# xguo7/SND-VAE

Measured on AMD Instinct MI355X. Metric: training graphs/sec + ELBO-step ms, N=4096 d=64, at 1/2/4/8 MI355X, higher is better.
Workload: dtype bf16; 1 GPU; C2: node-latent SND-VAE train step, N=4096, d=64, 8 graphs/GPU, HIP-graph replay; n_nodes=4096, latent=64, graphs_per_gpu=8, global_batch=8, parallelism=dp1, hip_graph=True

## Files before the change

snd_vae_amd/csrc/snd_common.hpp:

```cpp
#pragma once
#include <hip/hip_runtime.h>
#include <cstdint>
#include <cstdio>
#include <string>

#include "../../include/snd_vae.h"

namespace snd {

void set_error(const char* fmt, ...);

#define SND_CHECK_ARG(cond, ...)                                   \
  do {                                                             \
    if (!(cond)) {                                                 \
      ::snd::set_error(__VA_ARGS__);                               \
      return SND_ERR_ARG;                                          \
    }                                                              \
  } while (0)

#define SND_LAUNCH_CHECK(what)                                     \
  do {                                                             \
    hipError_t e_ = hipGetLastError();                             \
    if (e_ != hipSuccess) {                                        \
      ::snd::set_error("%s: %s", what, hipGetErrorString(e_));     \
// ... 25 lines not shown
inline int device_cu_count() {
  static const int n = [] {
    int d = 0, v = 0;
    if (hipGetDevice(&d) != hipSuccess ||
        hipDeviceGetAttribute(&v, hipDeviceAttributeMultiprocessorCount, d) != hipSuccess || v <= 0) {
      (void)hipGetLastError();
      return 256;
    }
    return v;
  }();
  return n;
}

__device__ __forceinline__ void edge_ce_terms(float x, float pw, float& coef, float& loss) {
  coef = -pw;
  if (pw != 1.f) {
    const float e = __expf(-fabsf(x));
    const float q = 1.f + e;
    const float r = __builtin_amdgcn_rcpf(q);
    const float sg = x >= 0.f ? r : e * r;
    coef += (pw - 1.f) * sg;
    loss += (pw - 1.f) * (fmaxf(x, 0.f) + __logf(q));
  }
}

__device__ __forceinline__ float kl_elem(float s, float mu) {
  const float x = 2.f * s;
  float r;
  if (fabsf(x) < 0.5f) {
    float t = 1.f / 3628800.f;
    t = __fmaf_rn(t, x, 1.f / 362880.f);
    t = __fmaf_rn(t, x, 1.f / 40320.f);
    t = __fmaf_rn(t, x, 1.f / 5040.f);
    t = __fmaf_rn(t, x, 1.f / 720.f);
    t = __fmaf_rn(t, x, 1.f / 120.f);
    t = __fmaf_rn(t, x, 1.f / 24.f);
    t = __fmaf_rn(t, x, 1.f / 6.f);
    t = __fmaf_rn(t, x, 0.5f);
    r = __fmul_rn(__fmul_rn(x, x), t);
  } else {
    r = __fsub_rn(__fsub_rn(__expf(x), 1.f), x);
  }
  return __fsub_rn(-r, __fmul_rn(mu, mu));
}

typedef __bf16 bf16x8 __attribute__((ext_vector_type(8)));
typedef __bf16 bf16x4 __attribute__((ext_vector_type(4)));
typedef float f32x4 __attribute__((ext_vector_type(4)));
typedef float f32x16 __attribute__((ext_vector_type(16)));
typedef unsigned u32x4 __attribute__((ext_vector_type(4)));

__device__ __forceinline__ float wave_sum(float v) {
#pragma unroll
  for (int o = 32; o > 0; o >>= 1) v += __shfl_xor(v, o, 64);
  return v;
}
__device__ __forceinline__ double wave_sum_d(double v) {
#pragma unroll
  for (int o = 32; o > 0; o >>= 1) v += __shfl_xor(v, o, 64);
  return v;
}
__device__ __forceinline__ unsigned wave_sum_u(unsigned v) {
#pragma unroll
  for (int o = 32; o > 0; o >>= 1) v += __shfl_xor(v, o, 64);
  return v;
}

template <int CTRL>
__device__ __forceinline__ float dpp_f(float v) {
  return __int_as_float(__builtin_amdgcn_update_dpp(0, __float_as_int(v), CTRL, 0xF, 0xF, true));
}
__device__ __forceinline__ float row8_sum(float v) {
  v += dpp_f<0xB1>(v);
  v += dpp_f<0x4E>(v);
  v += dpp_f<0x141>(v);
  return v;
}
__device__ __forceinline__ float row16_sum(float v) {
  v = row8_sum(v);
  v += dpp_f<0x140>(v);
  return v;
}

__device__ __forceinline__ uint4 philox4x32_10(uint4 c, uint2 k) {
  const unsigned M0 = 0xD2511F53u, M1 = 0xCD9E8D57u, W0 = 0x9E3779B9u, W1 = 0xBB67AE85u;
#pragma unroll
  for (int i = 0; i < 10; ++i) {
    const unsigned hi0 = __umulhi(M0, c.x), lo0 = M0 * c.x;
    const unsigned hi1 = __umulhi(M1, c.z), lo1 = M1 * c.z;
    c = make_uint4(hi1 ^ c.y ^ k.x, lo1, hi0 ^ c.w ^ k.y, lo0);
    k.x += W0;
    k.y += W1;
  }
  return c;
}

__device__ __forceinline__ float4 philox_normal4(unsigned long long seed, unsigned offset,
                                                unsigned long long q) {
  const uint4 r = philox4x32_10(make_uint4((unsigned)q, (unsigned)(q >> 32), offset, 0u),
                                make_uint2((unsigned)seed, (unsigned)(seed >> 32)));
  const float k = 2.3283064365386963e-10f;
  const float m1 = __builtin_amdgcn_sqrtf(-2.0f * __logf(((float)r.x + 1.0f) * k));
  const float m2 = __builtin_amdgcn_sqrtf(-2.0f * __logf(((float)r.z + 1.0f) * k));
  float s1, c1, s2, c2;
  __sincosf(6.283185307179586f * ((float)r.y * k), &s1, &c1);
  __sincosf(6.283185307179586f * ((float)r.w * k), &s2, &c2);
  return make_float4(m1 * c1, m1 * s1, m2 * c2, m2 * s2);
}

__device__ __forceinline__ float philox_normal(unsigned long long seed, unsigned offset,
                                               unsigned long long idx) {
  const float4 v = philox_normal4(seed, offset, idx >> 2);
  switch (idx & 3) {
    case 0: return v.x;
    case 1: return v.y;
    case 2: return v.z;
    default: return v.w;
  }
}

__device__ __forceinline__ void reparam_bwd_elem(float mu, float ls, float eps, float djd, float ej, float dzd,
                                                 float adj, float kl, float& dm, float& dl) {
  const float es = __expf(ls);
  const float dz = __fmaf_rn(adj, __fadd_rn(djd, ej), dzd);
  dm = __fmaf_rn(kl, mu, dz);
  dl = __fmaf_rn(__fmul_rn(dz, eps), es, __fmul_rn(kl, __fmaf_rn(es, es, -1.f)));
}

inline int cdiv(long long a, long long b) { return (int)((a + b - 1) / b); }
inline long long round_up(long long a, long long b) { return (a + b - 1) / b * b; }

__device__ __forceinline__ void adam_elem(float& p, float& m, float& v, float g, float b1, float b2,
                                          float eps, float lrt) {
  m = __fmaf_rn(b1, m, __fmul_rn(1.f - b1, g));
  v = __fmaf_rn(b2, v, __fmul_rn(__fmul_rn(1.f - b2, g), g));
  p = __fsub_rn(p, __fmul_rn(__fmul_rn(lrt, m),
                             __builtin_amdgcn_rcpf(__fadd_rn(__builtin_amdgcn_sqrtf(v), eps))));
}

}
```

snd_vae_amd/csrc/snd_elem.hip:

```cpp
#include "snd_elem.hpp"

#include <algorithm>
#include "snd_gemm.hpp"
#include "snd_tref.hpp"

namespace snd {
namespace {

template <typename T>
__device__ __forceinline__ T block_sum(T v) {
  __shared__ T sh[16];
  v = (sizeof(T) == 8) ? (T)wave_sum_d((double)v) : (T)wave_sum((float)v);
  const int w = threadIdx.x >> 6, nw = blockDim.x >> 6;
  if ((threadIdx.x & 63) == 0) sh[w] = v;
  __syncthreads();
  T t = 0;
  if (threadIdx.x == 0)
    for (int k = 0; k < nw; ++k) t += sh[k];
  return t;
}

constexpr int kReparamGrid = 2048;

__global__ void __launch_bounds__(256) reparam_fwd_kernel(ReparamFwdArgs a) {
// ... 261 lines not shown
#pragma unroll
      for (int k = 0; k < RG; ++k) {
        const int r = rb + k * RP;
        const bool rv = r < r1;
        dv[k] = rv ? a.dg[(long long)r * a.lddg + c] : 0.f;
        hv[k] = (rv && he) ? a.h2[(long long)r * a.ldh2 + c] : 0.f;
        pv[k] = (rv && hc) ? a.p[(long long)r * a.ldp + c] : 0.f;
      }
#pragma unroll
      for (int k = 0; k < RG; ++k) {
        const int r = rb + k * RP;
        if (r >= r1) break;
        float d = dv[k];
        if (he) {
          sge += d * hv[k];
          sbe += d;
          d *= gec;
        }
        if (hc) {
          sg += d * lrelu(pv[k]);
          sb += d;
          a.dp[(long long)r * a.lddp + c] = d * gc * lrelu_grad(pv[k]);
        }
      }
    }
  }
  if (a.has_enc) {
    sge = lane_rows_sum<CP>(sge, red);
    sbe = lane_rows_sum<CP>(sbe, red);
  }
  sg = lane_rows_sum<CP>(sg, red);
  sb = lane_rows_sum<CP>(sb, red);
  if (threadIdx.x < width) {
    const int stride = (a.has_enc ? 2 * a.wenc : 0) + 2 * a.h;
    float* pp = a.part + (long long)blockIdx.x * stride;
    int o = 0;
    if (a.has_enc) {
      pp[c] = sge * kBnC;
      pp[a.wenc + c] = sbe;
      o = 2 * a.wenc;
    }
    if (c < a.h) {
      pp[o + c] = sg * kBnC;
      pp[o + a.h + c] = sb;
    }
  }
}

#ifndef SND_RED_PL
#define SND_RED_PL 2
#endif
#ifndef SND_RED_PLS
#define SND_RED_PLS 4
#endif
#ifndef SND_RED_PLW
#define SND_RED_PLW 2
#endif
constexpr long long kRedWide = 2048;
__host__ __device__ __forceinline__ int red_pl(int nparts, long long items) {
  return nparts >= 1024 ? 64
                        : (nparts >= 256 ? 32 : (nparts >= 64 ? (items >= kRedWide ? SND_RED_PL : 8) : (items >= kRedWide ? SND_RED_PLW : SND_RED_PLS)));
}
struct ReducePack {
  ReduceDesc d[kMaxReduce];
  int bstart[kMaxReduce + 1];
};

template <int NTF> __device__ void finalize_block(const FinalizeArgs& a);

template <bool FIN, bool ADAM>
__global__ void __launch_bounds__(256) reduce_kernel(ReducePack pk, FinalizeArgs fin, ReduceAdam ra) {
  if constexpr (FIN) {
    if (blockIdx.x == 0) { finalize_block<256>(fin); return; }
  }
  const int bid = (int)blockIdx.x - (FIN ? 1 : 0);
  int di = 0;
#pragma unroll
  for (int i = 1; i < kMaxReduce; ++i) di += bid >= pk.bstart[i] ? 1 : 0;
  di = __builtin_amdgcn_readfirstlane(di);
  const ReduceDesc& d = pk.d[di];
  const int bx = bid - pk.bstart[di];
  const bool dad = ADAM && ((ra.mask >> di) & 1ull);
  float lrt = 0.f;
  if (dad) {
    const int st = *ra.stepn;
    lrt = (float)((double)ra.lr * sqrt(1.0 - pow((double)ra.b2, st)) / (1.0 - pow((double)ra.b1, st)));
  }
  __shared__ double red[256];
  const int rows = d.rows > 0 ? d.rows : 1;
  const long long items = (long long)rows * d.len;
  const int PL = red_pl(d.nparts, items);
  const int IPB = 256 / PL;
  const int it = threadIdx.x % IPB, pl = threadIdx.x / IPB;
  const long long j = (long long)bx * IPB + it;
  int r = 0, i = 0;
  double acc = 0.0;
  float pi = 0.f, mi = 0.f, vi = 0.f, prev = 0.f;
  if (j < items) {
    r = (int)(j / d.len);
    i = (int)(j - (long long)r * d.len);
    if (pl == 0) {
      const float* dst = d.dst + (long long)r * d.dst_rs + i;
      if (d.accumulate) prev = *dst;
      if constexpr (ADAM) {
        if (dad) {
          const long long k = dst - ra.gbase;
          pi = ra.p[k]; mi = ra.m[k]; vi = ra.v[k];
        }
      }
    }
    const float* src = d.src + (long long)r * d.src_rs + i;
    int p = pl;
    for (; p + 7 * PL < d.nparts; p += 8 * PL) {
      float v[8];
#pragma unroll
      for (int u = 0; u < 8; ++u) v[u] = src[(long long)(p + u * PL) * d.stride];
#pragma unroll
      for (int u = 0; u < 8; ++u) acc += (double)v[u];
    }
    for (; p + 3 * PL < d.nparts; p += 4 * PL) {
      const float v0 = src[(long long)p * d.stride];
      const float v1 = src[(long long)(p + PL) * d.stride];
      const float v2 = src[(long long)(p + 2 * PL) * d.stride];
      const float v3 = src[(long long)(p + 3 * PL) * d.stride];
      acc += (double)v0;
      acc += (double)v1;
      acc += (double)v2;
      acc += (double)v3;
    }
    for (; p < d.nparts; p += PL) acc += (double)src[(long long)p * d.stride];
  }
  red[threadIdx.x] = acc;
  __syncthreads();
  if (pl == 0 && j < items) {
    double t = 0.0;
    for (int q = 0; q < PL; ++q) t += red[q * IPB + it];
    float* dst = d.dst + (long long)r * d.dst_rs + i;
    float v = (float)(t * (double)d.scale);
    if (d.accumulate) v += prev;
    *dst = v;
    if constexpr (ADAM) {
      if (dad) {
        const long long k = dst - ra.gbase;
        adam_elem(pi, mi, vi, __fmul_rn(v, 1.f), ra.b1, ra.b2, ra.eps, lrt);
        ra.m[k] = mi;
        ra.v[k] = vi;
        ra.p[k] = pi;
      }
    }
  }
}

template <int NTF>
__device__ __forceinline__ void finalize_block(const FinalizeArgs& a) {
  double v[7] = {0, 0, 0, 0, 0, 0, 0};
#pragma unroll 4
  for (int k = threadIdx.x; k < a.n_zzt; k += NTF) { v[0] += a.zzt_part[2 * k]; v[1] += a.zzt_part[2 * k + 1]; }
#pragma unroll 4
  for (int k = threadIdx.x; k < a.n_edge; k += NTF) { v[2] += a.edge_part[2 * k]; v[3] += a.edge_part[2 * k + 1]; }
#pragma unroll 4
  for (int k = threadIdx.x; k < a.n_kl; k += NTF) v[4] += a.kl_part[k];
#pragma unroll 4
  for (int k = threadIdx.x; k < a.n_s; k += NTF) { v[5] += a.sse_s[k]; v[6] += a.sse_n[k]; }
  __shared__ double sh[NTF / 64][7];
#pragma unroll
  for (int q = 0; q < 7; ++q) v[q] = wave_sum_d(v[q]);
  if ((threadIdx.x & 63) == 0)
#pragma unroll
    for (int q = 0; q < 7; ++q) sh[threadIdx.x >> 6][q] = v[q];
  __syncthreads();
  double dl = 0, dc = 0, el = 0, tp = 0, kl = 0, ss = 0, sn = 0;
  if (threadIdx.x == 0)
    for (int w = 0; w < NTF / 64; ++w) {
      dl += sh[w][0]; dc += sh[w][1]; el += sh[w][2]; tp += sh[w][3];
      kl += sh[w][4]; ss += sh[w][5]; sn += sh[w][6];
    }
  if (threadIdx.x != 0) return;
  const double rows = (double)a.ngraphs * a.n;
  const double pairs = rows * (double)a.n;
  const double nnz = (double)a.rowptr[(long long)a.ngraphs * a.n];
  const double adj_sum = (double)a.norm * (dl + el + rows * kSoftplusM1);
  const double adj_cost = adj_sum / pairs;
  const double correct = pairs - nnz - dc + 2.0 * tp;
  const double klm = -0.5 * kl / (a.kl_count > 0 ? a.kl_count : rows * a.L);
  const double spatial = ss / (rows * a.sdim);
  const double node = sn / (rows * a.nfeat);
  const double cost = adj_cost + node + spatial + (double)a.beta * klm;
  double* L = a.losses;
  L[0] = cost; L[1] = spatial; L[2] = adj_cost; L[3] = node; L[4] = klm;
  L[5] = correct / pairs; L[6] = adj_sum; L[7] = correct;
  if (a.grad_tail)
    for (int k = 0; k < 6; ++k) a.grad_tail[k] = (float)L[k];
  if (a.step) *a.step += 1;
}

constexpr int kFinT = 1024;
__global__ void __launch_bounds__(kFinT) finalize_kernel(FinalizeArgs a) { finalize_block<kFinT>(a); }

__global__ void __launch_bounds__(256) adam_kernel(float* p, const float* g, float* m, float* v,
                                                   long long n, float lr, float b1, float b2,
                                                   float eps, float gscale, const int* step) {
  const int t = *step;
  const double lr_t = (double)lr * sqrt(1.0 - pow((double)b2, t)) / (1.0 - pow((double)b1, t));
  const float lrt = (float)lr_t;
  for (long long i = (long long)blockIdx.x * 256 + threadIdx.x; i < n;
       i += (long long)gridDim.x * 256) {
    float pi = p[i], mi = m[i], vi = v[i];
    adam_elem(pi, mi, vi, __fmul_rn(g[i], gscale), b1, b2, eps, lrt);
    m[i] = mi;
    v[i] = vi;
    p[i] = pi;
  }
}

}

int reparam_blocks(int rows, int L) {
  int b = cdiv((long long)rows * L, 256);
  return b < kReparamGrid ? (b < 1 ? 1 : b) : kReparamGrid;
}
int launch_reparam_fwd(const ReparamFwdArgs& a, hipStream_t s) {
  hipLaunchKernelGGL(reparam_fwd_kernel, dim3(reparam_blocks(a.rows, a.L)), dim3(256), 0, s, a);
  SND_LAUNCH_CHECK("reparam_fwd_kernel");
  return 0;
}
int launch_reparam_bwd(const ReparamBwdArgs& a, hipStream_t s) {
  hipLaunchKernelGGL(reparam_bwd_kernel, dim3(reparam_blocks(a.rows, a.L)), dim3(256), 0, s, a);
  SND_LAUNCH_CHECK("reparam_bwd_kernel");
  return 0;
}

bool small_head_supported(int rows, int gh, int L) {
  return rows >= 1 && rows <= kSmallHeadRows && rows * kSHC <= 256 && gh >= 1 && gh <= kSHK && L >= 1 &&
         2 * L <= kSHL2 && rows * kSHD <= 256;
}
int small_head_fwd_blocks(int L) { return cdiv(L, kSHC); }
int launch_small_head_fwd(const SmallHeadFwdArgs& a, hipStream_t s) {
  SND_CHECK_ARG(small_head_supported(a.rows, a.gh, a.L), "small_head: rows <= 16, gh <= 128, 2L <= 256");
  SND_CHECK_ARG(a.hh && a.wms && a.bms && a.ms && a.z && a.kl_part, "small_head_fwd: operands");
  hipLaunchKernelGGL(small_head_fwd_kernel, dim3(small_head_fwd_blocks(a.L)), dim3(256), 0, s, a);
  SND_LAUNCH_CHECK("small_head_fwd_kernel");
  return 0;
}
int launch_small_head_bwd(const SmallHeadBwdArgs& a, hipStream_t s) {
  SND_CHECK_ARG(small_head_supported(a.rows, a.gh, a.L), "small_head: rows <= 16, gh <= 128, 2L <= 256");
  SND_CHECK_ARG(a.hh && a.wms && a.ms && a.eps && a.dz && a.dms && a.slab && a.dh, "small_head_bwd: operands");
  hipLaunchKernelGGL(small_head_dms_kernel, dim3(cdiv(2 * a.L, kSHN)), dim3(256), 0, s, a);
  SND_LAUNCH_CHECK("small_head_dms_kernel");
  hipLaunchKernelGGL(small_head_dh_kernel, dim3(cdiv(a.gh, kSHD)), dim3(256), 0, s, a);
  SND_LAUNCH_CHECK("small_head_dh_kernel");
  return 0;
}

int head_blocks(int rows) { return cdiv(rows, kHeadRows); }

int launch_heads(const HeadArgs* h, int nheads, int rows, hipStream_t s) {
  if (nheads < 1 || nheads > 2) { set_error("heads: 1 or 2 heads"); return SND_ERR_ARG; }
  HeadPack pk{};
  for (int i = 0; i < nheads; ++i) {
    if (h[i].cin > kHeadK || h[i].cout > kHeadO) {
      set_error("heads: cin <= %d, cout <= %d", kHeadK, kHeadO);
      return SND_ERR_ARG;
    }
    pk.h[i] = h[i];
  }
  if (rows <= 0) return 0;
  hipLaunchKernelGGL(heads_kernel, dim3(head_blocks(rows), nheads), dim3(256), 0, s, pk, rows);
  SND_LAUNCH_CHECK("heads_kernel");
  return 0;
}

int col_blocks(int rows) { return cdiv(rows, kColRows); }

int launch_dec_bwd(const DecBwdArgs* a, int n, int rows, hipStream_t s) {
  if (n < 1 || n > 2) { set_error("dec_bwd: 1 or 2 descriptors"); return SND_ERR_ARG; }
  DecPack pk{};
  for (int i = 0; i < n; ++i) {
    if (a[i].ncols > 256) { set_error("dec_bwd: ncols %d > 256", a[i].ncols); return SND_ERR_ARG; }
    pk.d[i] = a[i];
  }
  if (rows <= 0) return 0;
  int w = a[0].ncols;
  if (n > 1 && a[1].ncols > w) w = a[1].ncols;
  dim3 grid(col_blocks(rows), n);
  if (w <= 16) hipLaunchKernelGGL(dec_bwd_kernel<16>, grid, dim3(256), 0, s, pk, rows);
  else if (w <= 32) hipLaunchKernelGGL(dec_bwd_kernel<32>, grid, dim3(256), 0, s, pk, rows);
  else if (w <= 64) hipLaunchKernelGGL(dec_bwd_kernel<64>, grid, dim3(256), 0, s, pk, rows);
// ... 134 lines not shown
```

snd_vae_amd/csrc/snd_fast.hpp:

```cpp
#pragma once
#include "snd_common.hpp"

namespace snd {

struct ColMap {
  int a, b, offb;
  __host__ __device__ int phys() const { return b ? offb + b : a; }
  __host__ __device__ bool valid(int c) const { return c < a || (b && c >= offb && c < offb + b); }
  __host__ __device__ int logical(int c) const { return c < a ? c : c - offb + a; }
};
inline ColMap colmap_plain(int n) { return {n, 0, n}; }
inline ColMap colmap_split(int a, int b) { return {a, b, (int)round_up(a, 8)}; }

struct PackSrc {
  const float* w;
  int A, B;
  int a0, a1, b0, b1;
  int n_off, k_off;
  int mode;
};
struct PackDesc {
  __bf16* dst;
  int T, kp, np;
  int nsrc;
  PackSrc s[2];
};
constexpr int kMaxPack = 16;
int launch_pack(const PackDesc* d, int n, hipStream_t s);
size_t pack_bytes(int T, int kp, int np);

enum RcEpi {
  RC_LIN = 0,
  RC_FWD = 1,
  RC_DECBWD = 2,
  RC_ENC1 = 3,
  RC_ENC0 = 4,
};
struct RcArgs {
  const void* x; int ldx; int K; int x_bf16;
  int R, npg, T;
  const __bf16* wpk; int kp, np;
  int N;
  ColMap cols;
  const float* bias; const float* gamma; const float* beta;
  const float* bias_b; const float* gamma_b; const float* beta_b;
  float* y; int ldy;
  void* out; int ldo; int out_bf16;
  float* colpart; int ncp;
  const float* p; int ldp;
  const float* xf; int ldxf; int f;
  const float* w0;
  const float* g2; const float* b2;
  int h;
  const void* zero;
  int dbg;
  int ktail; const float* wtail; int ldwt;
  int npb;
  const int* g_rowptr; const int* g_colidx; void* gout; int ldgo;
};
constexpr int kRcRows = 128;
constexpr size_t kRcLdsLimit = 136 * 1024;
int rc_blocks(int R);
size_t rc_lds_bytes(int T, int kp, int np);
int rc_cols_per_block(int T, int kp, int np);
int launch_rowconv(const RcArgs& a, int epi, hipStream_t s);

struct WgArgs {
  const void* x; int ldx; int K; int x_bf16;
  const void* dy; int lddy; int N; int dy_bf16;
  int R, npg, T;
  int rows_per_wg;
  int pairs_per_wg;
  float* slab;
  const void* zero;
  int dbg;
  int sK, sn4, wk0, wn0;
  unsigned* stamps;
  long long stamp_words;
};
struct WgGeom { int rows_per_wg, pairs_per_wg, gx, gy; };
WgGeom wgrad_geom(int R, int T, int K, int N, int chunks = 0);
inline int wgrad_n4(int N) { return (N + 3) & ~3; }
int launch_wgrad(const WgArgs& a, hipStream_t s);
constexpr int kMaxWgMulti = 32;
int launch_wgrad_multi(const WgArgs* a, int n, hipStream_t s);

struct HeadFastArgs {
  const void* u; int ldu; int u_bf16;
  const float* y; int ldy;
  const float* gamma; const float* beta;
  int cin;
  const float* w; const float* b; int cout;
  const float* target; int ldt;
  float count;
  float* yhat;
  __bf16* dy; int lddy;
  float* part;
  double* sse;
};
constexpr int kHeadFastRows = 256;
int heads_fast_blocks(int R);
bool heads_fast_supported(int cin, int cout);
int heads_fast_parts(int cin, int cout);
int launch_heads_fast(const HeadFastArgs* h, int n, int R, hipStream_t s);

struct Gcn0Args {
  const int* rowptr; const int* colidx; int R;
  const float* x; int ldx; int f;
  const float* w0; const float* g0; const float* b0; int h0;
  __bf16* h1; int ldh1;
  float* ax; __bf16* axb;
  int xcd_nbg;
  const int* row_order;
  PackDesc pack[kMaxPack]; int pack_blk[kMaxPack + 1]; int npack;
};
int xcd_nbg(int npg, int ngraphs);
int gcn0_blocks(int R);
int launch_gcn0(const Gcn0Args& a, hipStream_t s);

struct SpmmBfArgs {
  const int* rowptr; const int* colidx; int R;
  const __bf16* h; int ldh; int width; int epi;
  __bf16* out; int ldo;
  float* pre; int ldp;
  const float* g1; const float* b1;
  const float* x; int ldx; int f;
  const float* ge; const float* be;
  __bf16* g; int ldg;
  int xcd_nbg;
  const int* row_order;
  const int* t_rowid = nullptr; const int* t_trp = nullptr; const uint16_t* t_lcol = nullptr;
  const int* t_ucol = nullptr; int t_rows = 0; int t_ustride = 0;
  int npg = 0; int ngraphs = 0;
};
int launch_spmm_bf16(const SpmmBfArgs& a, hipStream_t s);

struct ReparamBwdFastArgs {
  const float* ms; int ldms; int R; int L;
  const float* eps; const float* dz_dec; const float* dJd; const float* ej;
  float adj_scale, kl_scale;
  __bf16* dms; int lddms;
  float* colpart;
  const float* dJd_extra = nullptr; int nextra = 0;
};
int reparam_bwd_fast_blocks(int R, int L);
int edge_reparam_blocks(int R);

struct ReparamPrepArgs {
  const float* ms; int ldms; int n, npad, ngraphs, L;
  const float* eps_in; unsigned long long seed; const int* step;
  float* z; float* eps_out; __bf16* zb;
  __bf16* jrow; __bf16* jt; float* colpart;
  double* kl_part;
  int stage_only;
  unsigned long long eps_base = 0;
  int* stepn = nullptr;
};
int reparam_prep_blocks(int ngraphs, int npad);

struct EdgeBfArgs {
  const int* rowptr; const int* colidx; int R;
  const __bf16* z; int d;
  float pos_weight;
  float* ej;
  double* part;
  int xcd_nbg;
  const int* row_order;
};
int edge_bf16_blocks(int R);
int launch_edge_bf16(const EdgeBfArgs& a, hipStream_t s);
int launch_reparam_prep(const ReparamPrepArgs& a, int dp, hipStream_t s);
int launch_reparam_bwd_fast(const ReparamBwdFastArgs& a, hipStream_t s);
int launch_edge_reparam_bwd(const EdgeBfArgs& e, const ReparamBwdFastArgs& a, hipStream_t s);

int fast_init_attributes();
int debug_flags();

}
```

snd_vae_amd/csrc/snd_fast_enc.hip:

```cpp
#include "snd_fast.hpp"
#include "snd_gather.hpp"
#include "snd_pack.hpp"

#include <algorithm>

namespace snd {
namespace {

constexpr int NT = 256;
constexpr int LPR = kLpr;
constexpr int RPB = NT / LPR;

__device__ __forceinline__ int row_of(const int* order, int rb, int R) {
  const int slot = rb * RPB + threadIdx.x / LPR;
  return (order && slot < R) ? order[slot] : slot;
}

__device__ __forceinline__ int xcd_rowblock(int b, int nbg) {
  if (nbg <= 0) return b;
  const int x = b & 7, s = b >> 3;
  const int gi = s / nbg, lb = s - gi * nbg;
  return (x + 8 * gi) * nbg + lb;
}

__global__ void __launch_bounds__(NT) gcn0_kernel(Gcn0Args a) {
  const int nrb = (a.R + RPB - 1) / RPB;
  if ((int)blockIdx.x >= nrb) {
    const int pb = blockIdx.x - nrb;
    int s = 0;
    while (s + 1 < a.npack && pb >= a.pack_blk[s + 1]) ++s;
    s = __builtin_amdgcn_readfirstlane(s);
    const PackDesc& d = a.pack[s];
    const int i = (pb - a.pack_blk[s]) * NT + threadIdx.x;
    if (i < pack_chunks(d)) pack_chunk(d, i);
    return;
  }
  __shared__ float sp[6][128];
  for (int i = threadIdx.x; i < a.h0; i += NT) {
#pragma unroll
    for (int q = 0; q < 4; ++q) sp[q][i] = q < a.f ? a.w0[q * a.h0 + i] : 0.f;
    sp[4][i] = a.g0[i] * kBnC;
    sp[5][i] = a.b0[i];
  }
  __syncthreads();
  const int sub = threadIdx.x & (LPR - 1);
  const int r = row_of(a.row_order, xcd_rowblock(blockIdx.x, a.xcd_nbg), a.R);
  const bool rv = r < a.R;
  float ax[4] = {0.f, 0.f, 0.f, 0.f};
  if (rv) {
    const int s = a.rowptr[r], e = a.rowptr[r + 1];
    int k = s + sub;
    for (; k + LPR < e; k += 2 * LPR) {
      const int c0 = a.colidx[k], c1 = a.colidx[k + LPR];
      float v0[4], v1[4];
#pragma unroll
      for (int j = 0; j < 4; ++j) {
        v0[j] = j < a.f ? a.x[(long long)c0 * a.ldx + j] : 0.f;
        v1[j] = j < a.f ? a.x[(long long)c1 * a.ldx + j] : 0.f;
      }
#pragma unroll
      for (int j = 0; j < 4; ++j) ax[j] += v0[j] + v1[j];
    }
    if (k < e) {
      const int c0 = a.colidx[k];
#pragma unroll
      for (int j = 0; j < 4; ++j) ax[j] += j < a.f ? a.x[(long long)c0 * a.ldx + j] : 0.f;
    }
  }
#pragma unroll
  for (int j = 0; j < 4; ++j) ax[j] = row8_sum(ax[j]);
  if (!rv) return;
  for (int c8 = sub; 8 * c8 < a.h0; c8 += LPR) {
    float o[8];
#pragma unroll
    for (int j = 0; j < 8; ++j) {
      const int col = 8 * c8 + j;
      float p = 0.f;
#pragma unroll
      for (int q = 0; q < 4; ++q) p += ax[q] * sp[q][col];
      o[j] = lrelu(p) * sp[4][col] + sp[5][col];
    }
    *reinterpret_cast<uint4*>(a.h1 + (long long)r * a.ldh1 + 8 * c8) = to_bf16x8(o);
  }
  if (sub == 0) {
    float xv[8];
#pragma unroll
    for (int j = 0; j < 8; ++j) xv[j] = j < a.f ? a.x[(long long)r * a.ldx + j] : 0.f;
    *reinterpret_cast<uint4*>(a.h1 + (long long)r * a.ldh1 + a.h0) = to_bf16x8(xv);
    *reinterpret_cast<float4*>(a.ax + (long long)r * 4) = make_float4(ax[0], ax[1], ax[2], ax[3]);
    const float axp[8] = {ax[0], ax[1], ax[2], ax[3], 0.f, 0.f, 0.f, 0.f};
    *reinterpret_cast<uint4*>(a.axb + (long long)r * 8) = to_bf16x8(axp);
  }
}

template <int EPI, int NQ>
__device__ __forceinline__ void spmm_row_epilogue(const SpmmBfArgs& a, int r, int sub,
                                                  const float (&acc)[NQ][8]) {
  const int nch = a.width >> 3;
#pragma unroll
  for (int q = 0; q < NQ; ++q) {
    if (sub + 8 * q >= nch) continue;
    const int col = 64 * q + 8 * sub;
    if constexpr (EPI == SND_SPMM_PLAIN) {
      *reinterpret_cast<uint4*>(a.out + (long long)r * a.ldo + col) = to_bf16x8(acc[q]);
    } else {
      float* pp = a.pre + (long long)r * a.ldp + col;
      *reinterpret_cast<float4*>(pp) = make_float4(acc[q][0], acc[q][1], acc[q][2], acc[q][3]);
      *reinterpret_cast<float4*>(pp + 4) = make_float4(acc[q][4], acc[q][5], acc[q][6], acc[q][7]);
      float g[8];
#pragma unroll
      for (int j = 0; j < 8; ++j) {
        const int c = col + j;
        const float b1 = lrelu(acc[q][j]) * (a.g1[c] * kBnC) + a.b1[c];
        g[j] = b1 * (a.ge[c] * kBnC) + a.be[c];
      }
      *reinterpret_cast<uint4*>(a.g + (long long)r * a.ldg + col) = to_bf16x8(g);
    }
  }
  if constexpr (EPI == SND_SPMM_GCN) {
    if (sub == 0) {
// ... 535 lines not shown
    if (row < a.n && c < L) {
      const long long gr = (long long)g * a.n + row;
      const long long i = gr * L + c;
      const float4 m = *reinterpret_cast<const float4*>(a.ms + gr * a.ldms + c);
      if (a.stage_only) {
        z[0] = m.x; z[1] = m.y; z[2] = m.z; z[3] = m.w;
      } else {
        const float4 ls = *reinterpret_cast<const float4*>(a.ms + gr * a.ldms + L + c);
        const float4 ep = a.eps_in ? *reinterpret_cast<const float4*>(a.eps_in + i)
                                   : philox_normal4(a.seed, off, (a.eps_base + (unsigned long long)i) >> 2);
        const float mu[4] = {m.x, m.y, m.z, m.w}, s[4] = {ls.x, ls.y, ls.z, ls.w};
        const float e[4] = {ep.x, ep.y, ep.z, ep.w};
#pragma unroll
        for (int t = 0; t < 4; ++t) {
          const float es = __expf(s[t]);
          z[t] = mu[t] + e[t] * es;
          kl += (double)kl_elem(s[t], mu[t]);
        }
        *reinterpret_cast<float4*>(a.z + i) = make_float4(z[0], z[1], z[2], z[3]);
        *reinterpret_cast<float4*>(a.eps_out + i) = ep;
      }
      bf16x4 zb;
#pragma unroll
      for (int t = 0; t < 4; ++t) zb[t] = (__bf16)z[t];
      *reinterpret_cast<bf16x4*>(a.zb + gr * L + c) = zb;
    }
    bf16x4 jb;
#pragma unroll
    for (int t = 0; t < 4; ++t) {
      tile[rr][c + t] = z[t];
      jb[t] = (__bf16)(z[t] * sc);
      stile[rr][c + t] = (float)jb[t];
    }
    *reinterpret_cast<bf16x4*>(a.jrow + ((long long)g * a.npad + row) * DP + c) = jb;
  }
  kl = wave_sum_d(kl);
  if ((threadIdx.x & 63) == 0) red[threadIdx.x >> 6] = kl;
  __syncthreads();
  if (threadIdx.x == 0 && a.kl_part) {
    double t = 0.0;
    for (int k = 0; k < NT / 64; ++k) t += red[k];
    a.kl_part[blockIdx.y * gridDim.x + blockIdx.x] = t;
  }
  if (threadIdx.x < DP) {
    float cs = 0.f;
    for (int rr = 0; rr < 64; ++rr) cs += stile[rr][threadIdx.x];
    a.colpart[((long long)g * (a.npad / 64) + rb) * DP + threadIdx.x] = cs;
  }
  for (int idx = threadIdx.x; idx < 16 * DP; idx += NT) {
    const int c = idx >> 4, r4 = 4 * (idx & 15);
    bf16x4 t;
#pragma unroll
    for (int u = 0; u < 4; ++u) t[u] = (__bf16)tile[r4 + u][c];
    *reinterpret_cast<bf16x4*>(a.jt + ((long long)g * DP + c) * a.npad + rb * 64 + r4) = t;
  }
}

}

int gcn0_blocks(int R) { return cdiv(R, RPB); }

int xcd_nbg(int npg, int ngraphs) {
  return (npg % RPB == 0 && ngraphs % 8 == 0) ? npg / RPB : 0;
}

int launch_gcn0(const Gcn0Args& a0, hipStream_t s) {
  if (a0.R <= 0) return 0;
  Gcn0Args a = a0;
  SND_CHECK_ARG(a.npack >= 0 && a.npack <= kMaxPack, "gcn0: at most %d packed images", kMaxPack);
  int pb = 0;
  for (int i = 0; i < a.npack; ++i) {
    const PackDesc& x = a.pack[i];
    SND_CHECK_ARG((x.kp == 32 || x.kp == 64 || x.kp == 128 || x.kp == 256) && x.np % 16 == 0 && x.np > 0 &&
                      x.T >= 1 && x.nsrc >= 1 && x.nsrc <= 2 && x.dst,
                  "gcn0: bad pack descriptor %d (kp %d np %d T %d)", i, x.kp, x.np, x.T);
    a.pack_blk[i] = pb;
    pb += cdiv(pack_chunks(x), NT);
  }
  a.pack_blk[a.npack] = pb;
  SND_CHECK_ARG(a.f >= 1 && a.f <= 4 && a.h0 % 8 == 0 && a.h0 <= 128 && a.ldh1 % 8 == 0 &&
                    a.ldh1 >= a.h0 + 8,
                "gcn0: f in 1..4, h0 %% 8 (<= 128), ldh1 >= h0 + 8");
  SND_CHECK_ARG(a.rowptr && a.x && a.w0 && a.g0 && a.b0 && a.h1 && a.ax && a.axb, "gcn0: null operand");
  hipLaunchKernelGGL(gcn0_kernel, dim3(gcn0_blocks(a.R) + pb), dim3(NT), 0, s, a);
  SND_LAUNCH_CHECK("gcn0_kernel");
  return 0;
}

template <typename K>
static int tile_lds_attr(K kern, int bytes) {
  return hipFuncSetAttribute(reinterpret_cast<const void*>(kern), hipFuncAttributeMaxDynamicSharedMemorySize,
                             bytes) == hipSuccess ? 0 : SND_ERR_HIP;
}

template <int EPI>
static int launch_spmm_bf16_epi(const SpmmBfArgs& a, bool two, hipStream_t s) {
  const bool gcn_small = EPI == SND_SPMM_GCN && a.t_rows > 0 && cdiv(a.R, a.t_rows) <= 4 * 512 &&
                         !(debug_flags() & 2048);
  if (a.t_rows > 0 && a.t_ustride <= TILE_CAP && !gcn_small) {
    static const int attr = tile_lds_attr(spmm_bf16_tiled_kernel<EPI, 1, 1>, tile_lds_bytes<1>()) |
                            tile_lds_attr(spmm_bf16_tiled_kernel<EPI, 1, 2>, tile_lds_bytes<1>()) |
                            tile_lds_attr(spmm_bf16_tiled_kernel<EPI, 2, 1>, tile_lds_bytes<2>()) |
                            tile_lds_attr(spmm_bf16_tiled_kernel<EPI, 2, 2>, tile_lds_bytes<2>());
    if (attr) { set_error("spmm_bf16_tiled: hipFuncSetAttribute failed"); return SND_ERR_HIP; }
    const int ntiles = cdiv(a.R, a.t_rows);
    const size_t lds = (size_t)(a.t_ustride + 1) * 256 * (two ? 2 : 1);
    const int tpg = (a.npg > 0 && a.npg % a.t_rows == 0 && a.ngraphs % 8 == 0 &&
                     (long long)a.npg * a.ngraphs == a.R) ? a.npg / a.t_rows : 0;
    const int per_cu = std::max(1, std::min(2, (160 * 1024) / (int)std::max<size_t>(lds, 1)));
    const int grid = std::min(ntiles, 256 * per_cu);
    const bool one = a.t_rows <= TG;
#define SND_TILED(NQ, RPG) \
  hipLaunchKernelGGL((spmm_bf16_tiled_kernel<EPI, NQ, RPG>), dim3(grid), dim3(TNT), lds, s, a, ntiles, tpg)
    if (two) { if (one) SND_TILED(2, 1); else SND_TILED(2, 2); }
    else { if (one) SND_TILED(1, 1); else SND_TILED(1, 2); }
#undef SND_TILED
    return 0;
  }
  SND_CHECK_ARG(a.colidx || a.R == 0, "spmm_bf16: colidx");
  dim3 grid(cdiv(a.R, RPB));
  if (two) hipLaunchKernelGGL((spmm_bf16_kernel<EPI, 2>), grid, dim3(NT), 0, s, a);
  else hipLaunchKernelGGL((spmm_bf16_kernel<EPI, 1>), grid, dim3(NT), 0, s, a);
  return 0;
}

int launch_spmm_bf16(const SpmmBfArgs& a, hipStream_t s) {
  if (a.R <= 0) return 0;
  SND_CHECK_ARG(a.width > 0 && a.width % 8 == 0 && a.width <= 128 && a.ldh % 8 == 0,
                "spmm_bf16: 0 < width %% 8 <= 128, ldh %% 8");
  SND_CHECK_ARG((long long)a.R * a.ldh * 2 < (1ll << 31), "spmm_bf16: rows x ldh beyond the 2 GB buffer range");
  SND_CHECK_ARG(a.t_rows >= 0 && a.t_rows <= TRPG * TG, "spmm_bf16: tile_rows <= 128");
  SND_CHECK_ARG(a.t_rows == 0 || (a.t_rowid && a.t_trp && a.t_lcol && a.t_ucol && a.t_ustride >= 0 &&
                                  a.t_ustride <= 65535),
                "spmm_bf16: row tiles need rows, trp, lcol, ucol and 0 <= ustride <= 65535");
  const bool two = a.width > 64;
  if (a.epi == SND_SPMM_PLAIN) {
    SND_CHECK_ARG(a.out && a.ldo % 8 == 0, "spmm_bf16: out");
    SND_TRY(launch_spmm_bf16_epi<SND_SPMM_PLAIN>(a, two, s));
  } else {
    SND_CHECK_ARG(a.pre && a.g && a.g1 && a.b1 && a.ge && a.be && a.x && a.f <= 8 &&
                      a.ldp % 4 == 0 && a.ldg % 8 == 0 && a.ldg >= a.width + 8,
                  "spmm_bf16: GCN operands");
    SND_TRY(launch_spmm_bf16_epi<SND_SPMM_GCN>(a, two, s));
  }
  SND_LAUNCH_CHECK("spmm_bf16_kernel");
  return 0;
}

int edge_bf16_blocks(int R) { return cdiv(R, RPB); }

int launch_edge_bf16(const EdgeBfArgs& a, hipStream_t s) {
  if (a.R <= 0) return 0;
  SND_CHECK_ARG(a.d % 8 == 0 && a.d <= 128 && a.z && a.ej && a.part && a.rowptr, "edge_bf16: operands");
  SND_CHECK_ARG((long long)a.R * a.d * 2 < (1ll << 31), "edge_bf16: rows x d beyond the 2 GB buffer range");
  if (a.d > 64) hipLaunchKernelGGL(edge_bf16_kernel<2>, dim3(edge_bf16_blocks(a.R)), dim3(NT), 0, s, a);
  else hipLaunchKernelGGL(edge_bf16_kernel<1>, dim3(edge_bf16_blocks(a.R)), dim3(NT), 0, s, a);
  SND_LAUNCH_CHECK("edge_bf16_kernel");
  return 0;
}

int reparam_prep_blocks(int ngraphs, int npad) { return ngraphs * (npad / 64); }

int launch_reparam_prep(const ReparamPrepArgs& a, int dp, hipStream_t s) {
  if (a.ngraphs <= 0) return 0;
  SND_CHECK_ARG(a.npad % 64 == 0 && a.L <= dp && a.L % 4 == 0 && a.ldms % 4 == 0,
                "reparam_prep: npad %% 64, L <= dp, L and ldms %% 4");
  SND_CHECK_ARG(a.ms && a.zb && a.jrow && a.jt && a.colpart &&
// ... 77 lines not shown
```

snd_vae_amd/csrc/snd_gemm.hpp:

```cpp
#pragma once
#include "snd_common.hpp"

namespace snd {

constexpr int kGemmBK = 64;

enum AMode { A_ROW = 0, A_COL = 1, A_CONV = 2, A_CONVT = 3 };
enum BMode { B_ROW = 0, B_COL = 1, B_FLIP = 2 };
enum Epi { E_STORE = 0, E_CONV = 1, E_PART = 2 };

struct GemmArgs {
  int M, N, K;
  const float* A; int lda; int a_cin; int a_npg;
  const float* B; int ldb; int b_cout;
  float* C; int ldc;
  const float* bias; const float* gamma; const float* beta;
  float* pre; int ldp;
  int kchunk;
  int accumulate;
  int a_ones_m1;
};

int launch_gemm(GemmArgs g, int amode, int bmode, int epi, int dtype, int splits,
                hipStream_t s);
int gemm_splits(int K, int target_blocks_per_tile);

struct ReduceDesc {
  const float* src;
  float* dst;
  int nparts;
  int len;
  long long stride;
  float scale;
  int accumulate;
  int rows;
  long long src_rs, dst_rs;
};
constexpr int kMaxReduce = 48;
struct FinalizeArgs;
struct ReduceAdam {
  const float* gbase;
  float* p; float* m; float* v;
  float lr, b1, b2, eps;
  const int* stepn;
  unsigned long long mask;
};
int launch_reduce(const ReduceDesc* d, int n, hipStream_t s, const FinalizeArgs* fin = nullptr,
                  const ReduceAdam* adam = nullptr);

constexpr int kColRows = 64;

}
```

snd_vae_amd/csrc/snd_head.hip:

```cpp
#include "snd_head.hpp"
#include "snd_gather.hpp"
#include "snd_pack.hpp"

#include <algorithm>

namespace snd {
namespace {

constexpr int kHeadRows = 64;
constexpr int HWMAX = 16;
constexpr float kSqrtLog2e = 1.2011224087864498f;
__device__ __forceinline__ int cdiv_dev(int a, int b) { return (a + b - 1) / b; }

typedef __attribute__((address_space(1))) const void* gptr_t;
typedef __attribute__((address_space(3))) void* lptr_t;

__device__ __forceinline__ void hglds16(const void* g, void* lds) {
  __builtin_amdgcn_global_load_lds((gptr_t)g, (lptr_t)lds, 16, 0, 0);
}
__host__ __device__ __forceinline__ int hswz(int row, int kp) {
  return kp == 128 ? (row & 15) : (kp == 64 ? ((row >> 1) & 7) : 0);
}

struct FwdLay {
  int w2, w1, g, h, zt, total, sx_end;
  __host__ __device__ FwdLay(int HR, int kp1, int np1, int kp2, int np2, int L) {
    w2 = 0;
    w1 = np2 * kp2 * 2;
    g = w1 + np1 * kp1 * 2;
    h = g + HR * kp1 * 2;
    zt = h + HR * kp2 * 2;
    total = zt + HR * (L + 1) * 4;
    sx_end = 2 * HR * (L + 4) * 4;
  }
};
constexpr int kHeadStaticLds = 2 * 128 * 4 + 4 * 80 * 4 + 2 * HWMAX * 8;
constexpr int kHeadDynLds = 160 * 1024 - kHeadStaticLds - 512;

__device__ __forceinline__ void stage_img(const __bf16* src, int bytes, char* dst, int nw) {
  const int lane = threadIdx.x & 63, w = threadIdx.x >> 6;
  const char* g = reinterpret_cast<const char*>(src) + lane * 16;
  for (int j = w; j < (bytes >> 10); j += nw) hglds16(g + (j << 10), dst + (j << 10));
}

template <int NBH>
__device__ __forceinline__ void img_gemm(const __bf16* xs, const __bf16* ws, int kp, int np, int rb,
                                         int nb0, int li, int lg, f32x4 (&acc)[NBH]) {
  const int nbc = np >> 4;
#pragma unroll
  for (int i = 0; i < NBH; ++i) acc[i] = f32x4{0.f, 0.f, 0.f, 0.f};
  const int xrow = 16 * rb + li;
  const __bf16* xrp = xs + xrow * kp;
  const int xsw = hswz(xrow, kp), wsw = hswz(li, kp);
  const __bf16* wrp = ws + li * kp;
  const int kcs = kp >> 5;
  for (int ks = 0; ks < kcs; ++ks) {
    const int ch = 4 * ks + lg;
    const bf16x8 bx = *reinterpret_cast<const bf16x8*>(xrp + ((ch ^ xsw) << 3));
#pragma unroll
    for (int i = 0; i < NBH; ++i) {
      if (nb0 + i < nbc) {
        const bf16x8 aw = *reinterpret_cast<const bf16x8*>(wrp + 16 * (nb0 + i) * kp + ((ch ^ wsw) << 3));
        acc[i] = __builtin_amdgcn_mfma_f32_16x16x32_bf16(aw, bx, acc[i], 0, 0, 0);
      }
    }
  }
}

__device__ __forceinline__ bf16x4* img_at4(__bf16* img, int row, int n0, int kp) {
  return reinterpret_cast<bf16x4*>(img + row * kp + (((n0 >> 3) ^ hswz(row, kp)) << 3) + (n0 & 4));
}

template <int F, int N>
__device__ __forceinline__ void feat_row(const float* x, int ldx, long long c, float (&v)[N]) {
  struct __attribute__((packed, aligned(4))) Row { float f[F]; };
  const Row t = *reinterpret_cast<const Row*>(x + c * ldx);
#pragma unroll
  for (int j = 0; j < N; ++j) v[j] = j < F ? t.f[j < F ? j : 0] : 0.f;
}

template <int HR, int NB1, int NB2>
__global__ void __launch_bounds__(HR * 8) head_fwd_kernel(HeadFwdArgs a) {
  constexpr int HT = HR * 8, HW = HT / 64, NRB = HR / 16;
  extern __shared__ __attribute__((aligned(16))) char smem[];
  __shared__ float cb1[128], cb2[128];
  __shared__ float cbn[4][80];
  __shared__ double klw[2 * HWMAX];
  const FwdLay lay(HR, a.kp1, a.np1, a.kp2, a.np2, a.L);
  __bf16* w2s = reinterpret_cast<__bf16*>(smem + lay.w2);
  __bf16* w1s = reinterpret_cast<__bf16*>(smem + lay.w1);
  __bf16* gs = reinterpret_cast<__bf16*>(smem + lay.g);
  __bf16* hs = reinterpret_cast<__bf16*>(smem + lay.h);
  float* mx = reinterpret_cast<float*>(smem);
  float* sx = reinterpret_cast<float*>(smem + HR * (a.L + 4) * 4);
  float* zt = reinterpret_cast<float*>(smem + lay.zt);
  const int L = a.L, sxs = L + 4, zts = L + 1;
  const int tid = threadIdx.x, lane = tid & 63, w = tid >> 6;
  const int tpg = a.npad / HR;
  int tb = blockIdx.x;
  if (a.ngraphs % 8 == 0 && a.ngraphs > 0) {
    const int x = tb & 7, sq = tb >> 3;
    const int g8 = sq / tpg;
    tb = (x + 8 * g8) * tpg + (sq - g8 * tpg);
  }
  const int gi = tb / tpg, lt = tb - gi * tpg;
  const int lr0 = lt * HR;
  const long long gr0 = (long long)gi * a.npg;

  for (int i = tid; i < HR * a.kp2 / 8; i += HT) reinterpret_cast<uint4*>(hs)[i] = make_uint4(0u, 0u, 0u, 0u);
  const int rs = tid >> 3, sub = tid & 7;
  const int lr = lr0 + rs;
  const bool rv = lr < a.npg;
  const long long r = gr0 + lr;
  const long long rc = gr0 + min(lr, a.npg - 1);
  const int nch = a.h1 >> 3, kc1 = a.kp1 >> 3;
  const int xo = (sub == nch) ? 0 : (sub + 8 == nch ? 1 : -1);
  const int pc = tid & 127;
  const float bhv = a.bh[min(pc, a.gh - 1)], bmsv = a.bms[min(pc, 2 * L - 1)];
  const int bc1 = min(tid, a.h1 - 1), bce = min(tid, a.h1 + a.f - 1);
  const float g1v = a.g1[bc1], b1v = a.b1[bc1], gev = a.ge[bce], bev = a.be[bce];
  const int rp0 = a.rowptr[rc], rp1 = a.rowptr[rc + 1];
  float xown[8];
  switch (a.f) {
    case 1: feat_row<1, 8>(a.x, a.ldx, rc, xown); break;
    case 2: feat_row<2, 8>(a.x, a.ldx, rc, xown); break;
    case 3: feat_row<3, 8>(a.x, a.ldx, rc, xown); break;
    case 4: feat_row<4, 8>(a.x, a.ldx, rc, xown); break;
    case 5: feat_row<5, 8>(a.x, a.ldx, rc, xown); break;
    case 6: feat_row<6, 8>(a.x, a.ldx, rc, xown); break;
    case 7: feat_row<7, 8>(a.x, a.ldx, rc, xown); break;
    default: feat_row<8, 8>(a.x, a.ldx, rc, xown); break;
  }
  stage_img(a.wh_img, a.np1 * a.kp1 * 2, reinterpret_cast<char*>(w1s), HW);
  stage_img(a.wms_img, a.np2 * a.kp2 * 2, reinterpret_cast<char*>(w2s), HW);
  if (tid < 128) {
    cb1[tid] = tid < a.gh ? bhv : 0.f;
    cb2[tid] = tid < 2 * L ? bmsv : 0.f;
  }
  if (tid < 80) { cbn[0][tid] = g1v; cbn[1][tid] = b1v; cbn[2][tid] = gev; cbn[3][tid] = bev; }
  __builtin_amdgcn_s_waitcnt(0x0F70);
  __syncthreads();
  uint4 gdat = make_uint4(0u, 0u, 0u, 0u), gxv = make_uint4(0u, 0u, 0u, 0u);
  if (xo >= 0 && rv) {
    float gv[8];
#pragma unroll
    for (int j = 0; j < 8; ++j) {
      const int c = a.h1 + j;
      gv[j] = j < a.f ? xown[j] * (cbn[2][c] * kBnC) + cbn[3][c] : 0.f;
    }
    gxv = to_bf16x8(gv);
  }

  float acc[8];
#pragma unroll
  for (int j = 0; j < 8; ++j) acc[j] = 0.f;
  if (rv && !(kdbg(a.dbg) & 1)) {
    const __amdgpu_buffer_rsrc_t rsd = rows_rsrc(a.xw1, (long long)a.R * a.h1 * 2);
    gather_rows16<1>(a.colidx, rp0, rp1, rsd, 2u * a.h1, sub,
                     [&](int, const u32x4 (&v)[1], bool) { acc8v(acc, v[0]); });
  }
  if (sub < nch) {
    float gv[8];
#pragma unroll
    for (int j = 0; j < 8; ++j) {
      const int c = 8 * sub + j;
      const float b1 = lrelu(acc[j]) * (cbn[0][c] * kBnC) + cbn[1][c];
      gv[j] = b1 * (cbn[2][c] * kBnC) + cbn[3][c];
    }
    gdat = to_bf16x8(gv);
  }
  {
    const bool d0 = sub < nch, x0 = xo == 0, x1 = xo == 1;
    const uint4 v0 = make_uint4(d0 ? gdat.x : (x0 ? gxv.x : 0u), d0 ? gdat.y : (x0 ? gxv.y : 0u),
                                d0 ? gdat.z : (x0 ? gxv.z : 0u), d0 ? gdat.w : (x0 ? gxv.w : 0u));
    const uint4 v1 = make_uint4(x1 ? gxv.x : 0u, x1 ? gxv.y : 0u, x1 ? gxv.z : 0u, x1 ? gxv.w : 0u);
    if (sub < kc1) *reinterpret_cast<uint4*>(gs + rs * a.kp1 + ((sub ^ hswz(rs, a.kp1)) << 3)) = v0;
    if (sub + 8 < kc1) *reinterpret_cast<uint4*>(gs + rs * a.kp1 + (((sub + 8) ^ hswz(rs, a.kp1)) << 3)) = v1;
  }
  __syncthreads();
  if (rv && !(kdbg(a.dbg) & 8)) {
    if (sub < nch) {
      float* pp = a.p1 + r * a.h1 + 8 * sub;
      *reinterpret_cast<float4*>(pp) = make_float4(acc[0], acc[1], acc[2], acc[3]);
      *reinterpret_cast<float4*>(pp + 4) = make_float4(acc[4], acc[5], acc[6], acc[7]);
      *reinterpret_cast<uint4*>(a.g + r * a.ldg + 8 * sub) = gdat;
    }
    if (xo >= 0) *reinterpret_cast<uint4*>(a.g + r * a.ldg + a.h1) = gxv;
  }

  const int li = lane & 15, lg = lane >> 4, rb = w % NRB, half = w / NRB;
  const int row = 16 * rb + li, lrw = lr0 + row;
  const bool vrow = lrw < a.npg;
  const long long rr = gr0 + lrw;
  {
    f32x4 acc1[NB1];
    if (kdbg(a.dbg) & 16) { for (int i = 0; i < NB1; ++i) acc1[i] = f32x4{0.f, 0.f, 0.f, 0.f}; }
    else img_gemm<NB1>(gs, w1s, a.kp1, a.np1, rb, NB1 * half, li, lg, acc1);
#pragma unroll
    for (int i = 0; i < NB1; ++i) {
      const int n0 = 16 * (NB1 * half + i) + 4 * lg;
      if (n0 >= a.gh) continue;
      bf16x4 v4;
#pragma unroll
      for (int e = 0; e < 4; ++e) v4[e] = (__bf16)(acc1[i][e] + cb1[n0 + e]);
      *img_at4(hs, row, n0, a.kp2) = v4;
      if (vrow && !(kdbg(a.dbg) & 8)) *reinterpret_cast<bf16x4*>(a.hh + rr * a.gh + n0) = v4;
    }
  }
  __syncthreads();

  {
    f32x4 acc2[NB2];
    if (kdbg(a.dbg) & 16) { for (int i = 0; i < NB2; ++i) acc2[i] = f32x4{0.f, 0.f, 0.f, 0.f}; }
    else img_gemm<NB2>(hs, w2s, a.kp2, a.np2, rb, NB2 * half, li, lg, acc2);
    float o[NB2][4];
#pragma unroll
    for (int i = 0; i < NB2; ++i) {
      const int n0 = 16 * (NB2 * half + i) + 4 * lg;
#pragma unroll
      for (int e = 0; e < 4; ++e) o[i][e] = acc2[i][e] + cb2[n0 + e];
      if (vrow && !(kdbg(a.dbg) & 8))
        *reinterpret_cast<float4*>(a.ms + rr * (2 * L) + n0) = make_float4(o[i][0], o[i][1], o[i][2], o[i][3]);
    }
    __syncthreads();
#pragma unroll
    for (int i = 0; i < NB2; ++i) {
      const int n0 = 16 * (NB2 * half + i) + 4 * lg;
      *reinterpret_cast<float4*>((half ? sx : mx) + row * sxs + (n0 - half * L)) =
          make_float4(o[i][0], o[i][1], o[i][2], o[i][3]);
    }
  }
  __syncthreads();

  {
    const unsigned off = a.step ? (unsigned)(*a.step) : 0u;
    if (a.stepn && blockIdx.x == 0 && tid == 0) *a.stepn = (int)off + 1;
    const int nq = L >> 2;
    double kl[HR / 64];
#pragma unroll
    for (int h = 0; h < HR / 64; ++h) kl[h] = 0.0;
    for (int it = (kdbg(a.dbg) & 32) ? HR * nq : tid; it < HR * nq; it += HT) {
      const int zr = it / nq, c = 4 * (it - zr * nq);
      const int zl = lr0 + zr;
      float z4[4] = {0.f, 0.f, 0.f, 0.f};
      if (zl < a.npg) {
        const long long ie = (gr0 + zl) * L + c;
        const float4 m4 = *reinterpret_cast<const float4*>(mx + zr * sxs + c);
        const float4 s4 = *reinterpret_cast<const float4*>(sx + zr * sxs + c);
        const float4 ep = a.eps_in ? *reinterpret_cast<const float4*>(a.eps_in + ie)
                                   : philox_normal4(a.seed, off, (a.eps_base + (unsigned long long)ie) >> 2);
        const float mu[4] = {m4.x, m4.y, m4.z, m4.w}, s[4] = {s4.x, s4.y, s4.z, s4.w};
        const float e[4] = {ep.x, ep.y, ep.z, ep.w};
        double kq = 0.0;
#pragma unroll
        for (int t = 0; t < 4; ++t) {
          const float es = __expf(s[t]);
          z4[t] = mu[t] + e[t] * es;
          kq += (double)kl_elem(s[t], mu[t]);
        }
#pragma unroll
        for (int h = 0; h < HR / 64; ++h) kl[h] += (zr >> 6) == h ? kq : 0.0;
        if (!(kdbg(a.dbg) & 8)) {
          *reinterpret_cast<float4*>(a.z + ie) = make_float4(z4[0], z4[1], z4[2], z4[3]);
          *reinterpret_cast<float4*>(a.eps_out + ie) = ep;
          bf16x4 zb;
#pragma unroll
          for (int t = 0; t < 4; ++t) zb[t] = (__bf16)z4[t];
          *reinterpret_cast<bf16x4*>(a.zb + ie) = zb;
        }
      }
      bf16x4 jb;
#pragma unroll
      for (int t = 0; t < 4; ++t) {
        jb[t] = (__bf16)(z4[t] * kSqrtLog2e);
        zt[zr * zts + c + t] = z4[t];
      }
      *reinterpret_cast<bf16x4*>(a.jrow + ((long long)gi * a.npad + zl) * L + c) = jb;
    }
#pragma unroll
    for (int h = 0; h < HR / 64; ++h) {
      const double v = wave_sum_d(kl[h]);
      if (lane == 0) klw[h * HWMAX + w] = v;
    }
  }
  __syncthreads();
  for (int i = (kdbg(a.dbg) & 64) ? HT * HR : tid; i < (HR / 64) * L; i += HT) {
    const int h = i / L, c = i - h * L;
    float cs = 0.f;
    for (int q0 = 0; q0 < 64; q0 += 16) {
      float t[16];
#pragma unroll
      for (int u = 0; u < 16; ++u) t[u] = zt[(64 * h + q0 + u) * zts + c];
#pragma unroll
      for (int u = 0; u < 16; ++u) cs += (float)(__bf16)(t[u] * kSqrtLog2e);
    }
    a.colpart[((long long)gi * (a.npad / 64) + (HR / 64) * lt + h) * L + c] = cs;
  }
  for (int idx = (kdbg(a.dbg) & 64) ? HT * HR : tid; idx < (HR / 4) * L; idx += HT) {
    const int c = idx / (HR / 4), r4 = 4 * (idx % (HR / 4));
    bf16x4 t;
#pragma unroll
    for (int u = 0; u < 4; ++u) t[u] = (__bf16)zt[(r4 + u) * zts + c];
    *reinterpret_cast<bf16x4*>(a.jt + ((long long)gi * L + c) * a.npad + lr0 + r4) = t;
  }
  if (tid < HR / 64) {
    double v = 0.0;
    for (int k = 0; k < HW; ++k) v += klw[tid * HWMAX + k];
    a.kl_part[(long long)gi * (a.npad / 64) + (HR / 64) * lt + tid] = v;
  }
}

template <int HR, int NB1, int NB2>
int head_fwd_launch(const HeadFwdArgs& a, hipStream_t s) {
  const size_t lds = (size_t)FwdLay(HR, a.kp1, a.np1, a.kp2, a.np2, a.L).total;
  hipLaunchKernelGGL((head_fwd_kernel<HR, NB1, NB2>), dim3(a.ngraphs * (a.npad / HR)), dim3(HR * 8), lds, s, a);
  SND_LAUNCH_CHECK("head_fwd_kernel");
  return 0;
}
template <int HR>
int head_fwd_dispatch(const HeadFwdArgs& a, hipStream_t s) {
  const int nb1 = (a.np1 / 16 + 1) / 2, nb2 = a.np2 / 32;
  if (nb1 == 1) return nb2 == 2 ? head_fwd_launch<HR, 1, 2>(a, s) : head_fwd_launch<HR, 1, 4>(a, s);
  return nb2 == 2 ? head_fwd_launch<HR, 2, 2>(a, s) : head_fwd_launch<HR, 2, 4>(a, s);
}

struct BwdLay {
  int w1, w2, m, h, red, total;
  __host__ __device__ BwdLay(int kp1, int np1, int kp2, int np2, int L, int hr = kHeadBwdRows) {
    w1 = 0;
    w2 = np1 * kp1 * 2;
    m = w2 + np2 * kp2 * 2;
    h = m + hr * kp1 * 2;
    red = h + hr * kp2 * 2;
    total = red + (hr / 8) * 2 * L * 4;
  }
};
constexpr int kBwdStaticLds = ((kHeadBwdRows / 16) * 4 * 128 + (kHeadBwdRows / 16) * 128 + 5 * 128) * 4 +
                              (kHeadBwdRows / 8) * 12;

__device__ __forceinline__ float shfl_rows8(float v) {
  v += __shfl_xor(v, 8, 64);
  v += __shfl_xor(v, 16, 64);
  v += __shfl_xor(v, 32, 64);
  return v;
}

template <int HR, int NQ, int NB1, int NB2>
__global__ void __launch_bounds__(HR * 8) head_bwd_kernel(HeadBwdArgs a) {
  constexpr int HT = HR * 8, HW = HT / 64, NRB = HR / 16;
  extern __shared__ __attribute__((aligned(16))) char smem[];
  __shared__ __attribute__((aligned(16))) float cps[NRB][4][128];
  __shared__ __attribute__((aligned(16))) float cpb[NRB][128];
  __shared__ float colp[5][128];
  __shared__ double sl[HW];
  __shared__ unsigned stp[HW];
  const BwdLay lay(a.kp1, a.np1, a.kp2, a.np2, a.L, HR);
  __bf16* w1s = reinterpret_cast<__bf16*>(smem + lay.w1);
  __bf16* w2s = reinterpret_cast<__bf16*>(smem + lay.w2);
  __bf16* ms_img = reinterpret_cast<__bf16*>(smem + lay.m);
  __bf16* dh_img = reinterpret_cast<__bf16*>(smem + lay.h);
  float* bred = reinterpret_cast<float*>(smem + lay.red);
  const int L = a.L, L2 = 2 * L;
  const int tid = threadIdx.x, lane = tid & 63, w = tid >> 6;
  int t = blockIdx.x;
  if (a.ngraphs % 8 == 0 && a.npg % HR == 0 && a.ngraphs > 0) {
    const int tpg = a.npg / HR, x = t & 7, sq = t >> 3;
    const int gi = sq / tpg;
    t = (x + 8 * gi) * tpg + (sq - gi * tpg);
  }
  const int r0 = t * HR;

  for (int i = tid; i < HR * a.kp2 / 8; i += HT) reinterpret_cast<uint4*>(dh_img)[i] = make_uint4(0u, 0u, 0u, 0u);
  const int pn = min(tid, 127);
  const float pge = a.ge[min(pn, a.W - 1)], pg1 = a.g1[min(pn, a.h1 - 1)], pb1 = a.b1[min(pn, a.h1 - 1)];

  {
    const int rs = tid >> 3, sub = tid & 7;
    const int r = r0 + rs;
    const bool rv = r < a.R;
    const int nch = L >> 3;
    bool qv[NQ];
#pragma unroll
    for (int q = 0; q < NQ; ++q) qv[q] = sub + 8 * q < nch;
    float lossr = 0.f;
    unsigned tp = 0;
    u32x4 zi[NQ];
// ... 232 lines not shown
      for (int q = 0; q < 4; ++q) {
        float v[4];
#pragma unroll
        for (int e = 0; e < 4; ++e) v[e] = row16_sum(qs[q][e]);
        if (li == 0) *reinterpret_cast<float4*>(&cps[rb][q][n0]) = make_float4(v[0], v[1], v[2], v[3]);
      }
    }
  }
  __syncthreads();
  for (int i = tid; i < 4 * a.W; i += HT) {
    const int q = i / a.W, n = i - q * a.W;
    float v = 0.f;
#pragma unroll
    for (int b = 0; b < NRB; ++b) v += cps[b][q][n];
    a.enc1_part[(long long)t * 4 * a.W + i] = v;
  }
}

template <int NQ, int NB1, int NB2>
int head_bwd_launch(const HeadBwdArgs& a, hipStream_t s) {
  const int hr = head_bwd_rows(a.R);
  const size_t lds = (size_t)BwdLay(a.kp1, a.np1, a.kp2, a.np2, a.L, hr).total;
  if (hr == kHeadBwdTinyRows)
    hipLaunchKernelGGL((head_bwd_kernel<kHeadBwdTinyRows, NQ, NB1, NB2>), dim3(head_tiles(a.R)),
                       dim3(kHeadBwdTinyRows * 8), lds, s, a);
  else if (hr == 64)
    hipLaunchKernelGGL((head_bwd_kernel<64, NQ, NB1, NB2>), dim3(head_tiles(a.R)), dim3(64 * 8), lds, s, a);
  else
    hipLaunchKernelGGL((head_bwd_kernel<kHeadBwdRows, NQ, NB1, NB2>), dim3(head_tiles(a.R)),
                       dim3(kHeadBwdRows * 8), lds, s, a);
  SND_LAUNCH_CHECK("head_bwd_kernel");
  return 0;
}

template <int F>
__device__ __forceinline__ void front_ax(const float* x, int ldx, const int* colidx, int s, int e, int sub,
                                         int rc, float (&ax)[4], float (&xown)[4]) {
  feat_row<F, 4>(x, ldx, rc, xown);
  if (s >= e) return;
  const int last = e - 1;
  int c[4];
#pragma unroll
  for (int u = 0; u < 4; ++u) c[u] = colidx[min(s + sub + 8 * u, last)];
#pragma unroll
  for (int u = 0; u < 4; ++u) asm volatile("" : "+v"(c[u]));
  float v[4][4];
#pragma unroll
  for (int u = 0; u < 4; ++u) feat_row<F, 4>(x, ldx, c[u], v[u]);
#pragma unroll
  for (int u = 0; u < 4; ++u)
#pragma unroll
    for (int j = 0; j < F; ++j) asm volatile("" : "+v"(v[u][j]));
#pragma unroll
  for (int t = 0; t < 2; ++t) {
    const int k = s + sub + 16 * t;
    const bool p0 = k < e, p1 = k + 8 < e;
#pragma unroll
    for (int j = 0; j < 4; ++j) {
      const float v0 = p0 ? v[2 * t][j] : 0.f, v1 = p1 ? v[2 * t + 1][j] : 0.f;
      ax[j] += p1 ? v0 + v1 : v0;
    }
  }
  int k = s + sub + 32;
  for (; k + 8 < e; k += 16) {
    const int c0 = colidx[k], c1 = colidx[k + 8];
    float v0[4], v1[4];
    feat_row<F, 4>(x, ldx, c0, v0);
    feat_row<F, 4>(x, ldx, c1, v1);
#pragma unroll
    for (int j = 0; j < 4; ++j) ax[j] += v0[j] + v1[j];
  }
  if (k < e) {
    float v0[4];
    feat_row<F, 4>(x, ldx, colidx[k], v0);
#pragma unroll
    for (int j = 0; j < 4; ++j) ax[j] += v0[j];
  }
}

template <int NB>
__global__ void __launch_bounds__(1024) enc_front_kernel(FrontArgs a) {
  const int tid = threadIdx.x;
  const int ntiles = cdiv_dev(a.R, 128);
  if ((int)blockIdx.x >= ntiles) {
    const int pb = blockIdx.x - ntiles;
    int s = 0;
    while (s + 1 < a.npack && pb >= a.pack_wg[s + 1]) ++s;
    s = __builtin_amdgcn_readfirstlane(s);
    const PackDesc& d = a.pack[s];
    const int i = (pb - a.pack_wg[s]) * 1024 + tid;
    if (i < pack_chunks(d)) pack_chunk(d, i);
    return;
  }
  extern __shared__ __attribute__((aligned(16))) char smem[];
  __shared__ float sp[6][128];
  __bf16* wimg = reinterpret_cast<__bf16*>(smem);
  __bf16* himg = reinterpret_cast<__bf16*>(smem + a.np1 * a.kp1 * 2);
  const int r0 = blockIdx.x * 128;
  const int K1 = a.h0 + a.f;
  const int rs = tid >> 3, sub = tid & 7;
  const int r = r0 + rs;
  const bool rv = r < a.R;
  const int fm = a.f - 1;
  const int pi = min(tid, a.h0 - 1);
  float spv[6];
#pragma unroll
  for (int q = 0; q < 4; ++q) spv[q] = a.w0[min(q, fm) * a.h0 + pi];
  spv[4] = a.g0[pi];
  spv[5] = a.b0[pi];
  const int kc = a.kp1 >> 3;
  const bool w1one = a.np1 * kc <= 1024;
  const int wc = tid % kc, wn = tid / kc;
  const int wlc = wc ^ img_swz(wn, a.kp1);
  float w1v[8];
  if (w1one) {
    const int nn = min(wn, a.n1 - 1);
#pragma unroll
    for (int j = 0; j < 8; ++j) w1v[j] = a.w1[min(8 * wlc + j, K1 - 1) * a.n1 + nn];
  }
  const int rc = min(r, a.R - 1);
  const int s = a.rowptr[rc], e1 = a.rowptr[rc + 1];
  const int e = rv ? e1 : s;
  float ax[4] = {0.f, 0.f, 0.f, 0.f}, xown[4];
  switch (a.f) {
    case 1: front_ax<1>(a.x, a.ldx, a.colidx, s, e, sub, rc, ax, xown); break;
    case 2: front_ax<2>(a.x, a.ldx, a.colidx, s, e, sub, rc, ax, xown); break;
    case 3: front_ax<3>(a.x, a.ldx, a.colidx, s, e, sub, rc, ax, xown); break;
    default: front_ax<4>(a.x, a.ldx, a.colidx, s, e, sub, rc, ax, xown); break;
  }
#pragma unroll
  for (int j = 0; j < 4; ++j) asm volatile("" : "+v"(ax[j]));
  if (w1one)
#pragma unroll
    for (int j = 0; j < 8; ++j) asm volatile("" : "+v"(w1v[j]));
  if (tid < a.h0) {
#pragma unroll
    for (int q = 0; q < 4; ++q) sp[q][tid] = q < a.f ? spv[q] : 0.f;
    sp[4][tid] = spv[4] * kBnC;
    sp[5][tid] = spv[5];
  }
  __syncthreads();
#pragma unroll
  for (int j = 0; j < 4; ++j) ax[j] = row8_sum(ax[j]);
  const int nch = a.h0 >> 3, kc1 = a.kp1 >> 3;
  uint4 hd = make_uint4(0u, 0u, 0u, 0u), hx = make_uint4(0u, 0u, 0u, 0u);
  if (sub < nch) {
    float o[8];
#pragma unroll
    for (int j = 0; j < 8; ++j) {
      const int col = 8 * sub + j;
      float p = 0.f;
#pragma unroll
      for (int q = 0; q < 4; ++q) p += ax[q] * sp[q][col];
      o[j] = lrelu(p) * sp[4][col] + sp[5][col];
    }
    hd = to_bf16x8(o);
  }
  const int xo = (sub == nch) ? 0 : (sub + 8 == nch ? 1 : -1);
  if (xo >= 0 && rv) {
    float xv[8];
#pragma unroll
    for (int j = 0; j < 8; ++j) xv[j] = (j < 4 && j < a.f) ? xown[j & 3] : 0.f;
    hx = to_bf16x8(xv);
  }
  {
    const bool d0 = sub < nch, x0 = xo == 0, x1 = xo == 1;
    const uint4 v0 = make_uint4(d0 ? hd.x : (x0 ? hx.x : 0u), d0 ? hd.y : (x0 ? hx.y : 0u),
                                d0 ? hd.z : (x0 ? hx.z : 0u), d0 ? hd.w : (x0 ? hx.w : 0u));
    const uint4 v1 = make_uint4(x1 ? hx.x : 0u, x1 ? hx.y : 0u, x1 ? hx.z : 0u, x1 ? hx.w : 0u);
    if (sub < kc1) *reinterpret_cast<uint4*>(himg + rs * a.kp1 + ((sub ^ hswz(rs, a.kp1)) << 3)) = v0;
    if (sub + 8 < kc1) *reinterpret_cast<uint4*>(himg + rs * a.kp1 + (((sub + 8) ^ hswz(rs, a.kp1)) << 3)) = v1;
  }
  if (w1one) {
    if (tid < a.np1 * kc) {
      bf16x8 v;
#pragma unroll
      for (int j = 0; j < 8; ++j) v[j] = (__bf16)((8 * wlc + j < K1 && wn < a.n1) ? w1v[j] : 0.f);
      *reinterpret_cast<bf16x8*>(wimg + wn * a.kp1 + 8 * wc) = v;
    }
  } else {
    for (int i = tid; i < a.np1 * kc; i += 1024) {
      const int c = i % kc, n = i / kc;
      const int lc = c ^ img_swz(n, a.kp1);
      float wv[8];
#pragma unroll
      for (int j = 0; j < 8; ++j) wv[j] = a.w1[min(8 * lc + j, K1 - 1) * a.n1 + min(n, a.n1 - 1)];
      bf16x8 v;
#pragma unroll
      for (int j = 0; j < 8; ++j) v[j] = (__bf16)((8 * lc + j < K1 && n < a.n1) ? wv[j] : 0.f);
      *reinterpret_cast<bf16x8*>(wimg + n * a.kp1 + 8 * c) = v;
    }
  }
  if (rv && !(kdbg(a.dbg) & 8)) {
    if (sub < nch) *reinterpret_cast<uint4*>(a.h1 + (long long)r * a.ldh1 + 8 * sub) = hd;
    if (xo >= 0) *reinterpret_cast<uint4*>(a.h1 + (long long)r * a.ldh1 + a.h0) = hx;
    if (sub == 0) {
      *reinterpret_cast<float4*>(a.ax + (long long)r * 4) = make_float4(ax[0], ax[1], ax[2], ax[3]);
      const float axp[8] = {ax[0], ax[1], ax[2], ax[3], 0.f, 0.f, 0.f, 0.f};
      *reinterpret_cast<uint4*>(a.axb + (long long)r * 8) = to_bf16x8(axp);
    }
  }
  __syncthreads();
  const int lane = tid & 63, w = tid >> 6;
  const int li = lane & 15, lg = lane >> 4, rb = w & 7, half = w >> 3;
  const int row = 16 * rb + li, rr = r0 + row;
  f32x4 acc[NB];
  img_gemm<NB>(himg, wimg, a.kp1, a.np1, rb, NB * half, li, lg, acc);
  if (rr >= a.R || (kdbg(a.dbg) & 8)) return;
#pragma unroll
  for (int i = 0; i < NB; ++i) {
    const int n0 = 16 * (NB * half + i) + 4 * lg;
    if (n0 >= a.n1) continue;
    bf16x4 v4;
#pragma unroll
    for (int e = 0; e < 4; ++e) v4[e] = (__bf16)(acc[i][e] + 0.f);
    *reinterpret_cast<bf16x4*>(a.xw1 + (long long)rr * a.n1 + n0) = v4;
  }
}

}

bool front_supported(int f, int h0, int n1, int kp1, int np1) {
  return f >= 1 && f <= 4 && h0 % 8 == 0 && h0 >= 8 && h0 <= 64 && h0 + 8 <= kp1 && n1 % 16 == 0 &&
         np1 == n1 && np1 <= 128 && (kp1 == 32 || kp1 == 64 || kp1 == 128) &&
         (np1 + 128) * kp1 * 2 + 6 * 128 * 4 <= 160 * 1024;
}

int launch_front(FrontArgs& a, const PackDesc* pack, int npack, hipStream_t s) {
  if (a.R <= 0) return 0;
  SND_CHECK_ARG(front_supported(a.f, a.h0, a.n1, a.kp1, a.np1), "front: unsupported widths (f %d h0 %d n1 %d)",
                a.f, a.h0, a.n1);
  SND_CHECK_ARG(npack >= 0 && npack <= kMaxPack, "front: at most %d packed images", kMaxPack);
  SND_CHECK_ARG(a.rowptr && (a.colidx || a.R == 0) && a.x && a.w0 && a.g0 && a.b0 && a.h1 && a.ax && a.axb &&
                    a.w1 && a.xw1 && a.ldh1 % 8 == 0 && a.ldh1 >= a.h0 + 8,
                "front: operands");
  a.npack = npack;
  int wg = 0;
  for (int i = 0; i < npack; ++i) {
    const PackDesc& x = pack[i];
    SND_CHECK_ARG((x.kp == 32 || x.kp == 64 || x.kp == 128) && x.np % 16 == 0 && x.np > 0 && x.T >= 1 &&
                      x.nsrc >= 1 && x.nsrc <= 2,
                  "front: bad pack descriptor %d", i);
    a.pack[i] = x;
    a.pack_wg[i] = wg;
    wg += cdiv(pack_chunks(x), 1024);
  }
  a.pack_wg[npack] = wg;
  SND_TRY(head_init_attributes());
  const size_t lds = (size_t)(a.np1 + 128) * a.kp1 * 2;
  const dim3 grid(cdiv(a.R, 128) + wg);
  switch ((a.np1 / 16 + 1) / 2) {
    case 1: hipLaunchKernelGGL((enc_front_kernel<1>), grid, dim3(1024), lds, s, a); break;
    case 2: hipLaunchKernelGGL((enc_front_kernel<2>), grid, dim3(1024), lds, s, a); break;
    case 3: hipLaunchKernelGGL((enc_front_kernel<3>), grid, dim3(1024), lds, s, a); break;
    default: hipLaunchKernelGGL((enc_front_kernel<4>), grid, dim3(1024), lds, s, a); break;
  }
  SND_LAUNCH_CHECK("enc_front_kernel");
  return 0;
}

int head_bwd_rows(int R) {
  if (cdiv(R, kHeadBwdRows) >= kHeadBwdSmall) return kHeadBwdRows;
  return cdiv(R, 64) < kHeadBwdTiny ? kHeadBwdTinyRows : 64;
}
int head_tiles(int R) { return cdiv(R, head_bwd_rows(R)); }

bool head_bwd_supported(int L, int gh, int W, int h1, int kp1, int np1, int kp2, int np2) {
  if ((L != 16 && L != 32 && L != 64) || kp1 != 2 * L) return false;
  if (gh % 16 || gh < 16 || np1 != gh || np1 > 64 || gh > kp2 || (kp2 != 32 && kp2 != 64 && kp2 != 128)) return false;
  if (W > 128 || np2 != (int)round_up(W, 16) || h1 % 4 || h1 < 4 || h1 > W) return false;
  return BwdLay(kp1, np1, kp2, np2, L).total + kBwdStaticLds <= 160 * 1024;
}

int launch_head_bwd(const HeadBwdArgs& a, hipStream_t s) {
  if (a.R <= 0) return 0;
  SND_CHECK_ARG(head_bwd_supported(a.L, a.gh, a.W, a.h1, a.kp1, a.np1, a.kp2, a.np2),
                "head_bwd: unsupported widths (L %d gh %d W %d h1 %d)", a.L, a.gh, a.W, a.h1);
  SND_CHECK_ARG((long long)a.R * a.L * 2 < (1ll << 31), "head_bwd: rows x L beyond the 2 GB buffer range");
  SND_CHECK_ARG((reinterpret_cast<uintptr_t>(a.p1) & 15) == 0, "head_bwd: P1 must be 16-byte aligned");
  SND_CHECK_ARG(a.rowptr && (a.colidx || a.R == 0) && a.zb && a.edge_part && a.ms && a.eps && a.dz_dec &&
                    a.dJd && a.dms && a.bms_part && a.wmsb_img && a.dh && a.bh_part && a.whb_img && a.ge &&
                    a.g1 && a.b1 && a.p1 && a.x && a.dp1 && a.enc1_part,
                "head_bwd: null operand");
  SND_TRY(head_init_attributes());
  const int nb1 = (a.np1 / 16 + 1) / 2, nb2 = (a.np2 / 16 + 1) / 2;
#define SND_HB(B1)                                   \
  switch (nb2) {                                     \
    case 1: return head_bwd_launch<1, B1, 1>(a, s);  \
    case 2: return head_bwd_launch<1, B1, 2>(a, s);  \
    case 3: return head_bwd_launch<1, B1, 3>(a, s);  \
    default: return head_bwd_launch<1, B1, 4>(a, s); \
  }
  if (nb1 == 1) { SND_HB(1) } else { SND_HB(2) }
#undef SND_HB
}

bool head_fwd_supported(int h1, int f, int gh, int L, int kp1, int np1, int kp2, int np2) {
  if (h1 % 8 || h1 < 8 || h1 > 64 || f < 1 || f > 8) return false;
  if ((kp1 != 32 && kp1 != 64 && kp1 != 128) || (kp2 != 32 && kp2 != 64 && kp2 != 128)) return false;
  if (h1 + 8 > kp1 || gh % 16 || gh < 16 || np1 != gh || np1 > 64 || gh > kp2) return false;
  if ((L != 32 && L != 64) || np2 != 2 * L) return false;
  const FwdLay l64(64, kp1, np1, kp2, np2, L), l128(128, kp1, np1, kp2, np2, L);
  return l128.total <= kHeadDynLds && l64.sx_end <= l64.zt && l128.sx_end <= l128.zt;
}

int launch_head_fwd(const HeadFwdArgs& a, hipStream_t s) {
  if (a.R <= 0) return 0;
  SND_CHECK_ARG(head_fwd_supported(a.h1, a.f, a.gh, a.L, a.kp1, a.np1, a.kp2, a.np2),
                "head_fwd: unsupported widths (h1 %d f %d gh %d L %d)", a.h1, a.f, a.gh, a.L);
  SND_CHECK_ARG(a.npad % 128 == 0 && a.npad >= a.npg && (long long)a.npg * a.ngraphs == a.R,
                "head_fwd: npad %% 128, R = ngraphs x npg");
  SND_CHECK_ARG(a.ldg % 8 == 0 && a.ldg >= a.h1 + 8, "head_fwd: ldg");
  SND_CHECK_ARG((long long)a.R * a.h1 * 2 < (1ll << 31), "head_fwd: rows x h1 beyond the 2 GB buffer range");
  SND_CHECK_ARG(a.rowptr && (a.colidx || a.R == 0) && a.xw1 && a.g1 && a.b1 && a.x && a.ge && a.be && a.p1 &&
                    a.g && a.wh_img && a.bh && a.hh && a.wms_img && a.bms && a.ms && a.z && a.eps_out &&
                    a.zb && a.jrow && a.jt && a.colpart && a.kl_part,
                "head_fwd: null operand");
  SND_TRY(head_init_attributes());
  return head_fwd_dispatch<kHeadRows>(a, s);
}

static int head_init_attributes_once() {
  const void* ks[] = {reinterpret_cast<const void*>(head_fwd_kernel<64, 1, 2>),
                      reinterpret_cast<const void*>(head_fwd_kernel<64, 1, 4>),
                      reinterpret_cast<const void*>(head_fwd_kernel<64, 2, 2>),
                      reinterpret_cast<const void*>(head_fwd_kernel<64, 2, 4>)};
  const void* kb[] = {reinterpret_cast<const void*>(head_bwd_kernel<kHeadBwdRows, 1, 1, 1>),
                      reinterpret_cast<const void*>(head_bwd_kernel<kHeadBwdRows, 1, 1, 2>),
                      reinterpret_cast<const void*>(head_bwd_kernel<kHeadBwdRows, 1, 1, 3>),
                      reinterpret_cast<const void*>(head_bwd_kernel<kHeadBwdRows, 1, 1, 4>),
                      reinterpret_cast<const void*>(head_bwd_kernel<kHeadBwdRows, 1, 2, 1>),
                      reinterpret_cast<const void*>(head_bwd_kernel<kHeadBwdRows, 1, 2, 2>),
                      reinterpret_cast<const void*>(head_bwd_kernel<kHeadBwdRows, 1, 2, 3>),
// ... 51 lines not shown
```

snd_vae_amd/csrc/snd_head.hpp:

```cpp
#pragma once
#include "snd_fast.hpp"

namespace snd {

struct HeadFwdArgs {
  const int* rowptr; const int* colidx;
  int R, npg, ngraphs, npad;
  const __bf16* xw1; int h1;
  const float* g1; const float* b1;
  const float* x; int ldx; int f;
  const float* ge; const float* be;
  float* p1;
  __bf16* g; int ldg;
  const __bf16* wh_img; int kp1, np1, gh;
  const float* bh;
  __bf16* hh;
  const __bf16* wms_img; int kp2, np2;
  const float* bms;
  float* ms;
  int L;
  const float* eps_in; unsigned long long seed; const int* step; unsigned long long eps_base;
  float* z; float* eps_out; __bf16* zb;
  __bf16* jrow; __bf16* jt; float* colpart;
  double* kl_part;
  int dbg;
  int* stepn = nullptr;
};
bool head_fwd_supported(int h1, int f, int gh, int L, int kp1, int np1, int kp2, int np2);
int launch_head_fwd(const HeadFwdArgs& a, hipStream_t s);

struct HeadBwdArgs {
  const int* rowptr; const int* colidx; int R;
  const __bf16* zb; int L; float pos_weight;
  double* edge_part;
  const float* ms; const float* eps; const float* dz_dec; const float* dJd;
  const float* dJd_extra; int nextra;
  float adj_scale, kl_scale;
  __bf16* dms; float* bms_part;
  const __bf16* wmsb_img; int kp1, np1, gh;
  __bf16* dh; float* bh_part;
  const __bf16* whb_img; int kp2, np2;
  int W, h1;
  const float* ge; const float* g1; const float* b1;
  const float* p1; const float* x; int ldx;
  __bf16* dp1; float* enc1_part;
  int npg, ngraphs;
  int dbg;
};
bool head_bwd_supported(int L, int gh, int W, int h1, int kp1, int np1, int kp2, int np2);
constexpr int kHeadBwdRows = 128;
#ifndef SND_HB_SMALL
#define SND_HB_SMALL 128
#endif
constexpr int kHeadBwdSmall = SND_HB_SMALL;
#ifndef SND_HB_TINY
#define SND_HB_TINY 128
#endif
#ifndef SND_HB_TINY_ROWS
#define SND_HB_TINY_ROWS 32
#endif
constexpr int kHeadBwdTinyRows = SND_HB_TINY_ROWS;
constexpr int kHeadBwdTiny = SND_HB_TINY;
int head_bwd_rows(int R);
int head_tiles(int R);
int launch_head_bwd(const HeadBwdArgs& a, hipStream_t s);

struct FrontArgs {
  const int* rowptr; const int* colidx; int R;
  const float* x; int ldx; int f;
  const float* w0; const float* g0; const float* b0; int h0;
  __bf16* h1; int ldh1; float* ax; __bf16* axb;
  const float* w1; int n1; int kp1, np1;
  __bf16* xw1;
  PackDesc pack[kMaxPack]; int npack;
  int pack_wg[kMaxPack + 1];
  int dbg;
};
bool front_supported(int f, int h0, int n1, int kp1, int np1);
int launch_front(FrontArgs& a, const PackDesc* pack, int npack, hipStream_t s);

int head_init_attributes();

}
```

snd_vae_amd/csrc/snd_step.hip:

```cpp
#include <algorithm>
#include <cstdarg>
#include <cstdlib>
#include <cstring>
#include <new>
#include <string>
#include <vector>

#include "snd_dec.hpp"
#include "snd_decode.hpp"
#include "snd_elem.hpp"
#include "snd_fast.hpp"
#include "snd_gemm.hpp"
#include "snd_head.hpp"
#include "snd_spmm.hpp"
#include "snd_tref.hpp"
#include "snd_sg.hpp"
#include "snd_zzt.hpp"

namespace snd {

static thread_local char g_err[512] = "";

void set_error(const char* fmt, ...) {
  va_list ap;
// ... 174 lines not shown
  SND_CHECK_ARG((long long)n_graphs * c.n_nodes < (1ll << 30), "snd_plan_create: batch too large");
  snd_plan* p = new (std::nothrow) snd_plan();
  if (!p) { set_error("snd_plan_create: out of memory"); return SND_ERR_ARG; }
  p->c = c;
  p->B = n_graphs; p->N = c.n_nodes; p->R = n_graphs * c.n_nodes;
  p->W = sg ? c.sg_h[5] : c.h1 + c.f_in;
  p->C1 = c.s1 + c.n1;
  p->tref = tref;
  p->sg = sg;
  p->S = sg ? c.sampling_num : 1;
  p->RS = (long long)n_graphs * p->S * c.n_nodes;
  p->dj = dj;
  p->RH = tref ? n_graphs * p->S : p->R;
  const int f = c.f_in, h0 = c.h0, h1 = c.h1, gh = c.g_hidden, L = c.latent;
  const int W = p->W, C1 = p->C1;
  const long long R = p->R, RH = p->RH;
  if (sg) {
    p->sgf[0] = f;
    p->sgf[1] = c.sg_h[2];
    p->add_block("enc.sg0", snd_sg_param_count(f, c.sg_h[0], c.sg_h[1], c.sg_h[2]));
    p->add_block("enc.sg1", snd_sg_param_count(c.sg_h[2], c.sg_h[3], c.sg_h[4], c.sg_h[5]));
  } else {
    p->add_block("enc.W0", (long long)f * h0);
    p->add_block("enc.bn0.gamma", h0);
    p->add_block("enc.bn0.beta", h0);
    p->add_block("enc.W1", (long long)(h0 + f) * h1);
    p->add_block("enc.bn1.gamma", h1);
    p->add_block("enc.bn1.beta", h1);
    p->add_block("enc.bne.gamma", W);
    p->add_block("enc.bne.beta", W);
  }
  p->add_block("enc.Wh", (tref ? (long long)p->N * W : W) * gh);
  p->add_block("enc.bh", gh);
  p->add_block("enc.Wms", (long long)gh * 2 * L);
  p->add_block("enc.bms", 2 * L);
  if (tref) {
    p->add_block("dec.Wp", (long long)L * p->N * dj);
    p->add_block("dec.bp", (long long)p->N * dj);
  }
  p->add_block("dec.K1", 5LL * dj * C1);
  p->add_block("dec.b1", C1);
  p->add_block("dec.bn1.gamma", C1);
  p->add_block("dec.bn1.beta", C1);
  p->add_block("dec.K2s", 5LL * c.s1 * c.s2);
  p->add_block("dec.b2s", c.s2);
  p->add_block("dec.bn2s.gamma", c.s2);
  p->add_block("dec.bn2s.beta", c.s2);
  p->add_block("dec.K2n", 5LL * c.n1 * c.n2);
  p->add_block("dec.b2n", c.n2);
  p->add_block("dec.bn2n.gamma", c.n2);
  p->add_block("dec.bn2n.beta", c.n2);
  p->add_block("dec.K3s", 5LL * c.s2 * c.s3);
  p->add_block("dec.b3s", c.s3);
  p->add_block("dec.bn3s.gamma", c.s3);
  p->add_block("dec.bn3s.beta", c.s3);
  p->add_block("dec.Ws", (long long)c.s3 * c.spatial_dim);
  p->add_block("dec.bs", c.spatial_dim);
  p->add_block("dec.Wn", (long long)c.n2 * c.num_feature);
  p->add_block("dec.bn", c.num_feature);

  p->add_buf("XW0", R * h0);  p->add_buf("P0", R * h0);  p->add_buf("H1", R * (h0 + f));
  p->add_buf("XW1", R * h1);  p->add_buf("P1", R * h1);  p->add_buf("H2", R * W);
  p->add_buf("G", R * W);     p->add_buf("Hh", RH * gh); p->add_buf("MS", RH * 2 * L);
  p->add_buf("EPS", RH * L);  p->add_buf("Z", R * dj);
  p->add_buf("ZSTAGE", (long long)zzt_staging_bytes(p->B, p->N, dj, c.dtype), 1);
  p->add_buf("DJD", R * dj);  p->add_buf("EJ", R * dj);
  p->add_buf("DJDX", std::max(1LL, (zzt_tsplit(p->B, p->N, c.dtype) - 1) * R * dj));
  p->add_buf("Y1", R * C1);   p->add_buf("U1", R * C1);
  p->add_buf("Y2S", R * c.s2); p->add_buf("U2S", R * c.s2);
  p->add_buf("Y2N", R * c.n2); p->add_buf("U2N", R * c.n2);
  p->add_buf("Y3S", R * c.s3); p->add_buf("U3S", R * c.s3);
  p->add_buf("SHAT", R * c.spatial_dim); p->add_buf("XHAT", R * c.num_feature);
  p->add_buf("DU3S", R * c.s3); p->add_buf("DY3S", R * c.s3);
  p->add_buf("DU2S", R * c.s2); p->add_buf("DY2S", R * c.s2);
  p->add_buf("DU2N", R * c.n2); p->add_buf("DY2N", R * c.n2);
  p->add_buf("DU1", R * C1);  p->add_buf("DY1", R * C1);  p->add_buf("DZDEC", R * dj);
  p->add_buf("DMS", RH * 2 * L); p->add_buf("DH", RH * gh); p->add_buf("DG", R * W);
  p->add_buf("DP1", R * h1);  p->add_buf("DXW1", R * h1); p->add_buf("DH1", R * h0);
  p->add_buf("DP0", R * h0);  p->add_buf("DXW0", R * h0);
  const int nz = zzt_dense_blocks(p->B, p->N, dj, c.dtype), ne = edge_blocks(p->R, dj);
  const int nk = reparam_blocks(p->RH, L), nh = head_blocks(p->R), nc = col_blocks(p->R);
  p->add_buf("PZZT", 2LL * nz, 8); p->add_buf("PEDGE", 2LL * std::max({ne, edge_bf16_blocks(p->R), head_tiles(p->R)}), 8); p->add_buf("PKL", std::max({nk, reparam_prep_blocks(p->B, zzt_npad(p->N)), small_head_fwd_blocks(c.latent)}), 8);
  p->add_buf("STEPN", 1);
  p->add_buf("PSSES", nh, 8); p->add_buf("PSSEN", nh, 8);
  p->add_buf("PHS", (long long)nh * (c.s3 * c.spatial_dim + c.spatial_dim));
  p->add_buf("PHN", (long long)nh * (c.n2 * c.num_feature + c.num_feature));
  p->add_buf("PDEC3", (long long)nc * 3 * c.s3); p->add_buf("PDEC2S", (long long)nc * 3 * c.s2);
  p->add_buf("PDEC2N", (long long)nc * 3 * c.n2); p->add_buf("PDEC1", (long long)nc * 3 * C1);
  p->add_buf("PENC1", (long long)nc * (2 * W + 2 * h1)); p->add_buf("PENC0", (long long)nc * 2 * h0);
  p->sW0 = wgrad_split(f, h0, p->R);
  p->sW1 = wgrad_split(h0 + f, h1, p->R);
  p->sWh = sg ? wgrad_split((int)std::min<long long>((long long)p->N * W + 1, 1 << 30), gh, (int)RH)
             : wgrad_split(W + 1, gh, p->R);
  p->sWms = wgrad_split(gh + 1, 2 * L, p->RH);
  p->small_head = tref && small_head_supported(p->RH, gh, L) && p->sWms.splits == 1;
  p->sK1 = wgrad_split(5 * dj, C1, p->R);
  p->sK2s = wgrad_split(5 * c.s1, c.s2, p->R);
  p->sK2n = wgrad_split(5 * c.n1, c.n2, p->R);
  p->sK3s = wgrad_split(5 * c.s2, c.s3, p->R);
  p->add_buf("SW0", (long long)p->sW0.splits * f * h0);
  p->add_buf("SW1", (long long)p->sW1.splits * (h0 + f) * h1);
  p->add_buf("SWH", (long long)p->sWh.splits * ((sg ? (long long)p->N * W : W) + 1) * gh);
  p->add_buf("SWMS", (long long)p->sWms.splits * (gh + 1) * 2 * L);
  p->add_buf("SK1", (long long)p->sK1.splits * 5 * dj * C1);
  if (sg) {
    const long long RS = p->RS, nnz = 2LL * (p->N - 1) * n_graphs * p->S;
    const int* h = c.sg_h;
    p->add_buf("SGLR", std::max(1LL, nnz)); p->add_buf("SGQ", std::max(1LL, nnz));
    p->add_buf("SGREV", std::max(1LL, nnz)); p->add_buf("SGDEG", RS); p->add_buf("SGE", RS);
    p->add_buf("SGBAD", 1);
    p->add_buf("SGY1", RS * h[2]); p->add_buf("SGX1", RS * h[2]); p->add_buf("SGDX1", RS * h[2]);
    p->add_buf("SGY2", RS * W);    p->add_buf("SGG", RS * W);      p->add_buf("SGDG", RS * W);
    p->add_buf("SGWS0", (long long)snd_sg_workspace((int)RS, f, h[0], h[1], h[2]), 1);
    p->add_buf("SGWS1", (long long)snd_sg_workspace((int)RS, h[2], h[3], h[4], h[5]), 1);
    p->add_buf("ZBAR", (long long)n_graphs * L); p->add_buf("DZBAR", (long long)n_graphs * L);
  }
  if (tref) {
    p->add_buf("ZL", RH * L);   p->add_buf("DZL", RH * L);
    p->add_buf("PHF", (long long)tref_head_fwd_blocks((long long)p->N * W, gh) * RH * gh);
    p->add_buf("PDZ", (long long)tref_proj_bwd_blocks((long long)p->N * dj) * RH * L);
  }
  p->add_buf("SK2S", (long long)p->sK2s.splits * 5 * c.s1 * c.s2);
  p->add_buf("SK2N", (long long)p->sK2n.splits * 5 * c.n1 * c.n2);
  p->add_buf("SK3S", (long long)p->sK3s.splits * 5 * c.s2 * c.s3);

  const int dbg = debug_flags();
#ifndef SND_WGC_SMALL
#define SND_WGC_SMALL 32
#endif
  const int wgc = (dbg & (4096 | 8192)) ? 0 : ((dbg & 16384) ? 32 : (R < 32768 ? SND_WGC_SMALL : 64));
  auto wgc_of = [&](int, int, int) { return wgc; };
  if (c.dtype == SND_BF16 && !sg && !(debug_flags() & 256)) {
    const ColMap m1 = colmap_split(c.s1, c.n1), m2 = colmap_split(c.s2, c.n2);
    const int w1 = m1.phys(), w2 = m2.phys();
    auto img = [&](int kin, int nout) {
      Img m{5, kp_of(kin), (int)round_up(nout, 16), 0};
      return m;
    };
    Img ims[6] = {img(dj, w1), img(w1, w2), img(c.s2, c.s3), img(c.s3, c.s2), img(w2, w1), img(w1, dj)};
    bool ok = heads_fast_supported(c.s3, c.spatial_dim) && heads_fast_supported(c.n2, c.num_feature) &&
              w1 <= 128;
    for (auto& m : ims)
      ok = ok && m.kp > 0 && m.np <= 128 && rc_cols_per_block(m.T, m.kp, m.np) > 0;
    if (ok) {
      p->fast = true;
      p->m1 = m1; p->m2 = m2;
#ifndef SND_LD_ALIGN
#define SND_LD_ALIGN 8
#endif
      p->ld1 = (int)round_up(w1, SND_LD_ALIGN); p->ld2 = (int)round_up(w2, SND_LD_ALIGN);
      p->ld3 = (int)round_up(c.s3, 8);
      const char* nm[6] = {"PK1F", "PK2F", "PK3F", "PK3B", "PK2B", "PK1B"};
      for (int i = 0; i < 6; ++i) {
        p->add_buf(nm[i], (long long)pack_bytes(ims[i].T, ims[i].kp, ims[i].np), 1);
        ims[i].off = p->bufs.back().off;
      }
      p->pk1f = ims[0]; p->pk2f = ims[1]; p->pk3f = ims[2];
      p->pk3b = ims[3]; p->pk2b = ims[4]; p->pk1b = ims[5];
      p->add_buf("ZERO", 64);
      p->add_buf("ZB", R * dj, 2);
      p->add_buf("FY1", R * p->ld1);    p->add_buf("FU1", R * p->ld1, 2);
      p->add_buf("FY2", R * p->ld2);    p->add_buf("FU2", R * p->ld2, 2);
      p->add_buf("FY3", R * p->ld3);    p->add_buf("FU3", R * p->ld3);
      p->add_buf("FDY3", R * p->ld3, 2); p->add_buf("FDY2", R * p->ld2, 2);
      p->add_buf("FDY1", R * p->ld1, 2);
      const int rcb = rc_blocks(p->R), hb = heads_fast_blocks(p->R);
// ... 134 lines not shown

extern "C" int snd_plan_set_option(snd_plan_t* p, const char* name, int value) {
  SND_CHECK_ARG(p && name, "snd_plan_set_option: bad args");
  if (!strcmp(name, "conc_decoder")) {
    p->conc_dec = value;
    set_zzt_splits(*p);
    return p->conc_dec_on() ? 1 : 0;
  }
  if (!strcmp(name, "reduce_adam")) {
    SND_CHECK_ARG(!p->fuse_m || (value != 0) == p->reduce_adam,
                  "snd_plan_set_option: reduce_adam cannot change while Adam is fused "
                  "(snd_plan_fuse_adam(plan, NULL, NULL, ...) first)");
    p->reduce_adam = value != 0;
    return p->reduce_adam ? 1 : 0;
  }
  set_error("snd_plan_set_option: unknown option '%s'", name);
  return SND_ERR_ARG;
}

void reduce_adam_cover(snd_plan& p);

extern "C" int snd_plan_fuse_adam(snd_plan_t* p, float* m, float* v, float lr, float beta1,
                                  float beta2, float eps) {
  SND_CHECK_ARG(p && ((m && v) || (!m && !v)), "snd_plan_fuse_adam: bad args");
  p->fuse_m = m; p->fuse_v = v;
  p->fuse_lr = lr; p->fuse_b1 = beta1; p->fuse_b2 = beta2; p->fuse_eps = eps;
  if (m && p->radam.empty()) reduce_adam_cover(*p);
  return 0;
}

extern "C" int snd_plan_set_rng_offset(snd_plan_t* p, long long head_row_offset) {
  SND_CHECK_ARG(p && head_row_offset >= 0, "snd_plan_set_rng_offset: bad args");
  p->rng_row0 = (unsigned long long)head_row_offset;
  return 0;
}

extern "C" int snd_plan_grad_event(snd_plan_t* p, int idx, void* event) {
  SND_CHECK_ARG(p && idx >= 0 && idx < (int)p->blocks.size(), "snd_plan_grad_event: bad index");
  const int pt = p->grad_point(p->blocks[idx].name);
  if (pt == 1) p->ev_proj = (hipEvent_t)event;
  if (pt == 2) p->ev_head = (hipEvent_t)event;
  return pt;
}
extern "C" int snd_plan_grad_event_get(const snd_plan_t* p, int idx, void** event) {
  SND_CHECK_ARG(p && event && idx >= 0 && idx < (int)p->blocks.size(), "snd_plan_grad_event_get: bad args");
  const int pt = p->grad_point(p->blocks[idx].name);
  *event = pt == 1 ? (void*)p->ev_proj : pt == 2 ? (void*)p->ev_head : nullptr;
  return pt;
}
extern "C" int snd_plan_block_fused(const snd_plan_t* p, int idx) {
  SND_CHECK_ARG(p && idx >= 0 && idx < (int)p->blocks.size(), "snd_plan_block_fused: bad index");
  return p->fused_kind((size_t)idx);
}
extern "C" int snd_plan_buffer(const snd_plan_t* p, const char* name, long long* off,
                               long long* numel) {
  SND_CHECK_ARG(p && name, "snd_plan_buffer: bad args");
  for (auto& b : p->bufs)
    if (b.name == name) {
      if (off) *off = b.off;
      if (numel) *numel = b.numel;
      return 0;
    }
  set_error("snd_plan_buffer: no buffer '%s'", name);
  return SND_ERR_ARG;
}

namespace {

struct Ctx {
  const snd_plan* p;
  char* ws;
  const float* P;
  float* Gr;
  hipStream_t s;
  hipStream_t side = nullptr;
  int* nev = nullptr;
  std::vector<WgArgs>* wq = nullptr;
  int zts = 1;
  float* f(const char* n) const { return (float*)(ws + p->buf(n)); }
  double* d(const char* n) const { return (double*)(ws + p->buf(n)); }
  const float* w(const char* n) const { return P + p->blk(n); }
  float* g(const char* n) const { return Gr + p->blk(n); }
  int* stepn() const { return reinterpret_cast<int*>(ws + p->buf("STEPN")); }
};

AdamFuse fused_adam(const Ctx& x, const char* blk, const int* step) {
  const snd_plan& p = *x.p;
  const long long o = p.blk(blk);
  return AdamFuse{const_cast<float*>(x.P) + o, p.fuse_m + o, p.fuse_v + o,
                  p.fuse_lr, p.fuse_b1, p.fuse_b2, p.fuse_eps, step};
}

int fork(const Ctx& x) {
  if (!x.side) return 0;
  SND_CHECK_ARG(*x.nev < snd_plan::kEvents, "train step: out of fork events");
  hipEvent_t e = x.p->ev[(*x.nev)++];
  if (hipEventRecord(e, x.s) != hipSuccess || hipStreamWaitEvent(x.side, e, 0) != hipSuccess) {
    set_error("train step: fork failed");
    return SND_ERR_HIP;
  }
  return 0;
}
int join(const Ctx& x) {
  if (!x.side) return 0;
  SND_CHECK_ARG(*x.nev < snd_plan::kEvents, "train step: out of join events");
  hipEvent_t e = x.p->ev[(*x.nev)++];
  if (hipEventRecord(e, x.side) != hipSuccess || hipStreamWaitEvent(x.s, e, 0) != hipSuccess) {
    set_error("train step: join failed");
    return SND_ERR_HIP;
  }
  return 0;
}
hipStream_t side(const Ctx& x) { return x.side ? x.side : x.s; }
int fork_to(const Ctx& x, hipStream_t o) {
  SND_CHECK_ARG(x.nev && *x.nev < snd_plan::kEvents, "train step: out of fork events");
  hipEvent_t e = x.p->ev[(*x.nev)++];
  if (hipEventRecord(e, x.s) != hipSuccess || hipStreamWaitEvent(o, e, 0) != hipSuccess) {
    set_error("train step: fork failed");
    return SND_ERR_HIP;
  }
  return 0;
}
int join_from(const Ctx& x, hipStream_t o) {
  SND_CHECK_ARG(x.nev && *x.nev < snd_plan::kEvents, "train step: out of join events");
  hipEvent_t e = x.p->ev[(*x.nev)++];
  if (hipEventRecord(e, o) != hipSuccess || hipStreamWaitEvent(x.s, e, 0) != hipSuccess) {
    set_error("train step: join failed");
    return SND_ERR_HIP;
  }
  return 0;
}
int wgrad(const Ctx& x, const WgArgs& a, hipStream_t s) {
  if (x.wq) { x.wq->push_back(a); return 0; }
  return launch_wgrad(a, s);
}
int mark(const Ctx& x) {
  if (!x.side) return -1;
  if (*x.nev >= snd_plan::kEvents) { set_error("train step: out of events"); return -2; }
  const int i = (*x.nev)++;
  if (hipEventRecord(x.p->ev[i], x.side) != hipSuccess) { set_error("train step: mark failed"); return -2; }
  return i;
}
int wait_mark(const Ctx& x, int i) {
  if (i == -1) return 0;
  if (i < 0 || hipStreamWaitEvent(x.s, x.p->ev[i], 0) != hipSuccess) {
    set_error("train step: wait failed");
    return SND_ERR_HIP;
  }
  return 0;
}

void init_concurrency(const snd_plan& p, hipStream_t main) {
  if (p.conc != 0) return;
  hipStreamCaptureStatus st = hipStreamCaptureStatusNone;
  if (hipStreamIsCapturing(main, &st) != hipSuccess || st != hipStreamCaptureStatusNone) return;
  p.conc = -1;
  if (hipStreamCreateWithFlags(&p.side, hipStreamNonBlocking) != hipSuccess) return;
  for (auto& e : p.ev)
    if (hipEventCreateWithFlags(&e, hipEventDisableTiming) != hipSuccess) return;
  p.conc = 1;
}

int gemm_fwd(const Ctx& x, int M, int N, int K, const float* A, int lda, const float* B, int ldb,
             int bmode, float* C, int ldc, const float* bias) {
  GemmArgs g{};
  g.M = M; g.N = N; g.K = K; g.A = A; g.lda = lda; g.B = B; g.ldb = ldb; g.C = C; g.ldc = ldc;
// ... 152 lines not shown
  const snd_config_t& c = p.c;
  const int L = c.latent, dj = p.dj, s1 = c.s1, n1 = c.n1, s2 = c.s2, n2 = c.n2, s3 = c.s3;
  const int C1 = p.C1;
  auto dst = [&](const Img& im) { return reinterpret_cast<__bf16*>(x.ws + im.off); };
  auto src = [](const float* w, int A, int B, int a0, int a1, int b0, int b1, int noff, int koff,
                int mode) { return PackSrc{w, A, B, a0, a1, b0, b1, noff, koff, mode}; };
  const float *K1 = x.w("dec.K1"), *K2s = x.w("dec.K2s"), *K2n = x.w("dec.K2n"), *K3s = x.w("dec.K3s");
  const int o1 = p.m1.offb, o2 = p.m2.offb;
  PackDesc d[6]{};
  d[0] = {dst(p.pk1f), 5, p.pk1f.kp, p.pk1f.np, 2,
          {src(K1, dj, C1, 0, dj, 0, s1, 0, 0, 0), src(K1, dj, C1, 0, dj, s1, C1, o1, 0, 0)}};
  d[1] = {dst(p.pk2f), 5, p.pk2f.kp, p.pk2f.np, 2,
          {src(K2s, s1, s2, 0, s1, 0, s2, 0, 0, 0), src(K2n, n1, n2, 0, n1, 0, n2, o2, o1, 0)}};
  d[2] = {dst(p.pk3f), 5, p.pk3f.kp, p.pk3f.np, 1, {src(K3s, s2, s3, 0, s2, 0, s3, 0, 0, 0), {}}};
  d[3] = {dst(p.pk3b), 5, p.pk3b.kp, p.pk3b.np, 1, {src(K3s, s2, s3, 0, s2, 0, s3, 0, 0, 1), {}}};
  d[4] = {dst(p.pk2b), 5, p.pk2b.kp, p.pk2b.np, 2,
          {src(K2s, s1, s2, 0, s1, 0, s2, 0, 0, 1), src(K2n, n1, n2, 0, n1, 0, n2, o1, o2, 1)}};
  d[5] = {dst(p.pk1b), 5, p.pk1b.kp, p.pk1b.np, 2,
          {src(K1, dj, C1, 0, dj, 0, s1, 0, 0, 1), src(K1, dj, C1, 0, dj, s1, C1, 0, o1, 1)}};
  for (int i = 0; i < 6; ++i) e[i] = d[i];
  if (!p.fast_enc) return 6;
  const int f = c.f_in, h0 = c.h0, h1 = c.h1, gh = c.g_hidden, W = p.W;
  auto one = [&](const Img& im, PackSrc ps) { return PackDesc{dst(im), 1, im.kp, im.np, 1, {ps, {}}}; };
  if (p.tref) {
    const float* W1 = x.w("enc.W1");
    e[6] = one(p.pw1f, src(W1, h0 + f, h1, 0, h0 + f, 0, h1, 0, 0, 0));
    e[7] = one(p.pw1b, src(W1, h0 + f, h1, 0, h0, 0, h1, 0, 0, 1));
    e[8] = one(p.pidg, src(nullptr, W, W, 0, W, 0, W, 0, 0, 2));
    return 9;
  }
  const float *W1 = x.w("enc.W1"), *Wh = x.w("enc.Wh"), *Wms = x.w("enc.Wms");
  e[6] = one(p.pw1f, src(W1, h0 + f, h1, 0, h0 + f, 0, h1, 0, 0, 0));
  e[7] = one(p.pwhf, src(Wh, W, gh, 0, W, 0, gh, 0, 0, 0));
  e[8] = one(p.pwmsf, src(Wms, gh, 2 * L, 0, gh, 0, 2 * L, 0, 0, 0));
  e[9] = one(p.pwmsb, src(Wms, gh, 2 * L, 0, gh, 0, 2 * L, 0, 0, 1));
  e[10] = one(p.pwhb, src(Wh, W, gh, 0, W, 0, gh, 0, 0, 1));
  e[11] = one(p.pw1b, src(W1, h0 + f, h1, 0, h0, 0, h1, 0, 0, 1));
  return 12;
}

int pack_decoder(const Ctx& x) {
  PackDesc e[kMaxPack]{};
  return launch_pack(e, build_packs(x, e), x.s);
}

static int spmm_bf16_plain(const snd_batch_t* batch, int R, int npg, int ngraphs, const __bf16* h,
                           int ldh, int width, __bf16* out, int ldo, hipStream_t s);

static void use_tiles(SpmmBfArgs& a, const snd_batch_t* batch, int npg, int ngraphs) {
  a.row_order = batch->row_order;
  if (batch->tiles.tile_rows <= 0) return;
  a.t_rowid = batch->tiles.rows; a.t_trp = batch->tiles.trp; a.t_lcol = batch->tiles.lcol;
  a.t_ucol = batch->tiles.ucol; a.t_rows = batch->tiles.tile_rows; a.t_ustride = batch->tiles.ustride;
  a.npg = npg; a.ngraphs = ngraphs;
}

static int spmm_bf16_plain(const snd_batch_t* batch, int R, int npg, int ngraphs, const __bf16* h,
                           int ldh, int width, __bf16* out, int ldo, hipStream_t s) {
  const snd_window_plan_t& w = batch->window;
  if (w.meta && width == 64 && w.beta >= 0 && ((w.beta + 7) & ~7) <= spmm_win_max_beta() &&
      !(debug_flags() & (1 << 22))) {
    SpmmWinArgs a{w.meta, w.slots, w.rows, w.order, w.beta, R, npg, ngraphs, h, ldh, width, out, ldo};
    return launch_spmm_window(a, s);
  }
  SpmmBfArgs a{batch->rowptr, batch->colidx, R, h, ldh, width, SND_SPMM_PLAIN, out, ldo};
  a.xcd_nbg = xcd_nbg(npg, ngraphs);
  use_tiles(a, batch, npg, ngraphs);
  return launch_spmm_bf16(a, s);
}

int encoder_fast_fwd(const Ctx& x, const snd_batch_t* batch) {
  const snd_plan& p = *x.p;
  const snd_config_t& c = p.c;
  const int R = p.R, L = c.latent, f = c.f_in, h0 = c.h0, h1 = c.h1, gh = c.g_hidden, W = p.W;
  auto bf = [&](const char* n) { return reinterpret_cast<__bf16*>(x.f(n)); };
  if (p.front_fused) {
    FrontArgs a{};
    a.rowptr = batch->rowptr; a.colidx = batch->colidx; a.R = R;
    a.x = batch->features; a.ldx = f; a.f = f;
    a.w0 = x.w("enc.W0"); a.g0 = x.w("enc.bn0.gamma"); a.b0 = x.w("enc.bn0.beta"); a.h0 = h0;
    a.h1 = bf("FH1"); a.ldh1 = p.ldh1; a.ax = x.f("AX"); a.axb = bf("AXB");
    a.w1 = x.w("enc.W1"); a.n1 = h1; a.kp1 = p.pw1f.kp; a.np1 = p.pw1f.np;
    a.xw1 = bf("FXW1"); a.dbg = debug_flags();
    PackDesc e[kMaxPack]{};
    const int ne = build_packs(x, e);
    SND_TRY(launch_front(a, e, ne, x.s));
  }
  if (!p.front_fused) {
    Gcn0Args a{batch->rowptr, batch->colidx, R, batch->features, f, f, x.w("enc.W0"),
               x.w("enc.bn0.gamma"), x.w("enc.bn0.beta"), h0, bf("FH1"), p.ldh1, x.f("AX"), bf("AXB"),
               xcd_nbg(p.N, p.B)};
    a.row_order = batch->row_order;
    if (p.pack_in_gcn0) a.npack = build_packs(x, a.pack);
    SND_TRY(launch_gcn0(a, x.s));
  }
  if (!p.front_fused) {
    RcArgs a = rc_args(p, x.ws, p.pw1f, bf("FH1"), p.ldh1, p.kw1, h1, colmap_plain(h1));
    a.ktail = h0 + f - p.kw1; a.wtail = x.w("enc.W1") + (long long)p.kw1 * h1; a.ldwt = h1;
    a.out = bf("FXW1"); a.ldo = h1; a.out_bf16 = 1;
    SND_TRY(launch_rowconv(a, RC_LIN, x.s));
  }
  if (p.head_fused) return 0;
  {
    SpmmBfArgs a{batch->rowptr, batch->colidx, R, bf("FXW1"), h1, h1, SND_SPMM_GCN, nullptr, 0,
                 x.f("FP1"), h1, x.w("enc.bn1.gamma"), x.w("enc.bn1.beta"), batch->features, f, f,
                 x.w("enc.bne.gamma"), x.w("enc.bne.beta"), bf("FG"), p.ldg, xcd_nbg(p.N, p.B)};
    use_tiles(a, batch, p.N, p.B);
    SND_TRY(launch_spmm_bf16(a, x.s));
  }
  if (p.tref) return 0;
  {
    RcArgs a = rc_args(p, x.ws, p.pwhf, bf("FG"), p.ldg, p.kwh, gh, colmap_plain(gh));
    a.ktail = W - p.kwh; a.wtail = x.w("enc.Wh") + (long long)p.kwh * gh; a.ldwt = gh;
    a.bias = x.w("enc.bh"); a.out = bf("FHH"); a.ldo = gh; a.out_bf16 = 1;
    SND_TRY(launch_rowconv(a, RC_LIN, x.s));
  }
  {
    RcArgs a = rc_args(p, x.ws, p.pwmsf, bf("FHH"), gh, gh, 2 * L, colmap_plain(2 * L));
    a.bias = x.w("enc.bms"); a.out = x.f("MS"); a.ldo = 2 * L; a.out_bf16 = 0;
    SND_TRY(launch_rowconv(a, RC_LIN, x.s));
  }
  return 0;
}

int head_fwd_fused(const Ctx& x, const snd_batch_t* batch, const float* eps, unsigned long long seed,
                   const int* step_counter, const ZztStage& stg) {
  const snd_plan& p = *x.p;
  const snd_config_t& c = p.c;
  HeadFwdArgs a{};
  a.rowptr = batch->rowptr; a.colidx = batch->colidx;
  a.R = p.R; a.npg = p.N; a.ngraphs = p.B; a.npad = zzt_npad(p.N);
  a.xw1 = reinterpret_cast<const __bf16*>(x.f("FXW1")); a.h1 = c.h1;
  a.g1 = x.w("enc.bn1.gamma"); a.b1 = x.w("enc.bn1.beta");
  a.x = batch->features; a.ldx = c.f_in; a.f = c.f_in;
  a.ge = x.w("enc.bne.gamma"); a.be = x.w("enc.bne.beta");
  a.p1 = x.f("FP1"); a.g = reinterpret_cast<__bf16*>(x.f("FG")); a.ldg = p.ldg;
  a.wh_img = reinterpret_cast<const __bf16*>(x.ws + p.pwhf.off); a.kp1 = p.pwhf.kp; a.np1 = p.pwhf.np;
  a.gh = c.g_hidden; a.bh = x.w("enc.bh"); a.hh = reinterpret_cast<__bf16*>(x.f("FHH"));
  a.wms_img = reinterpret_cast<const __bf16*>(x.ws + p.pwmsf.off); a.kp2 = p.pwmsf.kp; a.np2 = p.pwmsf.np;
  a.bms = x.w("enc.bms"); a.ms = x.f("MS"); a.L = c.latent;
  a.eps_in = eps; a.seed = seed; a.step = step_counter; a.eps_base = p.eps_base();
  a.z = x.f("Z"); a.eps_out = x.f("EPS"); a.zb = reinterpret_cast<__bf16*>(x.f("ZB"));
  a.jrow = reinterpret_cast<__bf16*>(stg.jrow); a.jt = reinterpret_cast<__bf16*>(stg.jt);
  a.colpart = stg.colpart; a.kl_part = x.d("PKL");
  a.stepn = x.stepn();
  a.dbg = debug_flags();
  return launch_head_fwd(a, x.s);
}

int encoder_fast_bwd_tail(const Ctx& x, const snd_batch_t* batch, bool enc1_done = false);

int head_bwd_fused(const Ctx& x, const snd_batch_t* batch, float adj_scale, float kl_scale) {
  const snd_plan& p = *x.p;
  const snd_config_t& c = p.c;
  const int R = p.R, L = c.latent, f = c.f_in, h1 = c.h1, gh = c.g_hidden, W = p.W;
  auto bf = [&](const char* n) { return reinterpret_cast<__bf16*>(x.f(n)); };
  {
    HeadBwdArgs a{};
    a.rowptr = batch->rowptr; a.colidx = batch->colidx; a.R = R;
    a.zb = bf("ZB"); a.L = L; a.pos_weight = c.pos_weight; a.edge_part = x.d("PEDGE");
    a.ms = x.f("MS"); a.eps = x.f("EPS"); a.dz_dec = x.f("DZDEC"); a.dJd = x.f("DJD");
    a.dJd_extra = x.f("DJDX"); a.nextra = x.zts - 1;
    a.adj_scale = adj_scale; a.kl_scale = kl_scale;
    a.dms = bf("FDMS"); a.bms_part = x.f("PHBMS");
    a.wmsb_img = reinterpret_cast<const __bf16*>(x.ws + p.pwmsb.off); a.kp1 = p.pwmsb.kp; a.np1 = p.pwmsb.np;
    a.gh = gh; a.dh = bf("FDH"); a.bh_part = x.f("PFBH");
    a.whb_img = reinterpret_cast<const __bf16*>(x.ws + p.pwhb.off); a.kp2 = p.pwhb.kp; a.np2 = p.pwhb.np;
    a.W = W; a.h1 = h1;
    a.ge = x.w("enc.bne.gamma"); a.g1 = x.w("enc.bn1.gamma"); a.b1 = x.w("enc.bn1.beta");
    a.p1 = x.f("FP1"); a.x = batch->features; a.ldx = f;
    a.dp1 = bf("FDP1"); a.enc1_part = x.f("PFENC1");
    a.npg = p.N; a.ngraphs = p.B; a.dbg = debug_flags();
    return launch_head_bwd(a, x.s);
  }
}

// ... 531 lines not shown
    dec("PDEC3", s3, "dec.bn3s.gamma", "dec.bn3s.beta", "dec.b3s");
    dec("PDEC2S", s2, "dec.bn2s.gamma", "dec.bn2s.beta", "dec.b2s");
    dec("PDEC2N", n2, "dec.bn2n.gamma", "dec.bn2n.beta", "dec.b2n");
    dec("PDEC1", C1, "dec.bn1.gamma", "dec.bn1.beta", "dec.b1");
    const int hs = s3 * sd + sd, hn = n2 * nf + nf;
    rd.push_back({x.f("PHS"), x.g("dec.Ws"), nh, s3 * sd, (long long)hs, 1.f, 0});
    rd.push_back({x.f("PHS") + s3 * sd, x.g("dec.bs"), nh, sd, (long long)hs, 1.f, 0});
    rd.push_back({x.f("PHN"), x.g("dec.Wn"), nh, n2 * nf, (long long)hn, 1.f, 0});
    rd.push_back({x.f("PHN") + n2 * nf, x.g("dec.bn"), nh, nf, (long long)hn, 1.f, 0});
  }
}

void reduce_adam_cover(snd_plan& p) {
  const uintptr_t wsb = (uintptr_t)1 << 44, gb = (uintptr_t)1 << 45;
  Ctx x{&p, (char*)wsb, (const float*)((uintptr_t)1 << 46), (float*)gb, nullptr};
  std::vector<ReduceDesc> rd;
  final_reduce_descs(x, rd);
  std::vector<unsigned char> hits((size_t)p.pcount, 0);
  std::vector<char> bad(p.blocks.size(), 0);
  for (const ReduceDesc& d : rd) {
    const long long o = d.dst - (float*)gb;
    const int rows = d.rows > 0 ? d.rows : 1;
    for (int r = 0; r < rows; ++r)
      for (int i = 0; i < d.len; ++i) {
        const long long k = o + (long long)r * d.dst_rs + i;
        if (k < 0 || k >= p.pcount) continue;
        if (hits[(size_t)k] < 2) ++hits[(size_t)k];
        if (d.accumulate) hits[(size_t)k] = 2;
      }
  }
  p.radam.assign(p.blocks.size(), 0);
  for (size_t b = 0; b < p.blocks.size(); ++b) {
    const Block& bl = p.blocks[b];
    if (p.stream_fused(bl.name) || bl.numel == 0) continue;
    bool ok = true;
    for (long long k = bl.off; k < bl.off + bl.numel && ok; ++k) ok = hits[(size_t)k] == 1;
    p.radam[b] = ok;
  }
}

unsigned long long reduce_adam_mask(const snd_plan& p, const std::vector<ReduceDesc>& rd, const float* G) {
  unsigned long long mask = 0;
  for (size_t i = 0; i < rd.size() && i < 64; ++i) {
    const long long o = rd[i].dst - G;
    for (size_t b = 0; b < p.blocks.size(); ++b)
      if (o >= p.blocks[b].off && o < p.blocks[b].off + p.blocks[b].numel && p.reduce_fused(b))
        mask |= 1ull << i;
  }
  return mask;
}

extern "C" int snd_train_step(const snd_plan_t* plan, const snd_batch_t* batch,
                              const float* params, float* grads, void* workspace,
                              const float* eps, unsigned long long seed, int* step_counter,
                              double* losses, snd_stream_t stream) {
  SND_CHECK_ARG(plan && batch && params && grads && workspace && losses,
                "snd_train_step: null argument");
  SND_CHECK_ARG(batch->rowptr && batch->colidx && batch->features && batch->feature_truth &&
                    batch->spatial_truth, "snd_train_step: incomplete batch");
  SND_TRY(zzt_init_attributes());
  const snd_plan& p = *plan;
  const snd_config_t& c = p.c;
  Ctx x{&p, (char*)workspace, params, grads, (hipStream_t)stream};
  p.last_params = params;
  p.last_grads = grads;
  int nev = 0;
  if (p.fast && (debug_flags() & 1024)) {
    init_concurrency(p, x.s);
    if (p.conc == 1) { x.side = p.side; x.nev = &nev; }
  }
  bool cdec = false;
  if (p.conc_dec_on() && !x.side) {
    init_concurrency(p, x.s);
    cdec = p.conc == 1;
    if (cdec) x.nev = &nev;
  }
  x.zts = cdec ? p.zzt_ts_conc : p.zzt_ts;
  p.last_zts = x.zts;
  std::vector<WgArgs> wq;
  if (p.fast && !x.side && !(debug_flags() & (4096 | 8192))) {
    wq.reserve(kMaxWgMulti);
    x.wq = &wq;
  }
  const int R = p.R, N = p.N, f = c.f_in, h0 = c.h0, h1 = c.h1, gh = c.g_hidden, L = c.latent;
  const int W = p.W, C1 = p.C1, s1 = c.s1, s2 = c.s2, s3 = c.s3, n1 = c.n1, n2 = c.n2;
  const int sd = c.spatial_dim, nf = c.num_feature;
  const int dj = p.dj, RH = p.RH;
  const long long KH = (long long)N * W, CP = (long long)N * dj;
  const int* rp = batch->rowptr;
  const int* ci = batch->colidx;
  const float* X = batch->features;
  if (p.fast) {
    SND_TRY(fast_init_attributes());
    if (!p.front_fused && !p.pack_in_gcn0) SND_TRY(pack_decoder(x));
  }

  if (p.sg) {
    SND_TRY(encoder_sg_fwd(x, batch));
  } else if (p.fast_enc) {
    SND_TRY(encoder_fast_fwd(x, batch));
  } else {
    SND_TRY(encoder_generic_fwd(x, batch));
  }
  if (p.fast_enc && p.tref) {
    TrefHeadFwdArgs a{nullptr, KH, p.B, x.w("enc.Wh"), gh, x.w("enc.bh"), x.f("PHF"),
                      reinterpret_cast<const __bf16*>(x.f("FG")), p.ldg, W, N};
    SND_TRY(launch_tref_head_fwd(a, x.s));
    const ReduceDesc rd{x.f("PHF"), x.f("Hh"), tref_head_fwd_blocks(KH, gh), RH * gh,
                        (long long)RH * gh, 1.f, 0, 0, 0, 0};
    SND_TRY(launch_reduce(&rd, 1, x.s));
    if (!p.small_head)
      SND_TRY(gemm_fwd(x, RH, 2 * L, gh, x.f("Hh"), gh, x.w("enc.Wms"), 2 * L, B_ROW, x.f("MS"), 2 * L,
                       x.w("enc.bms")));
  }
  const ZztStage stg = zzt_stage(x.ws + p.buf("ZSTAGE"), p.B, N, dj, c.dtype);
  if (p.tref) {
    if (p.small_head) {
      SmallHeadFwdArgs a{x.f("Hh"), RH, gh, x.w("enc.Wms"), x.w("enc.bms"), L, x.f("MS"), eps, seed,
                         step_counter, p.eps_base(), x.f("EPS"), x.f("ZL"), x.d("PKL")};
      a.stepn = x.stepn();
      SND_TRY(launch_small_head_fwd(a, x.s));
    } else {
      ReparamFwdArgs a{x.f("MS"), 2 * L, RH, L, eps, seed, step_counter, x.f("EPS"), x.f("ZL"),
                       x.d("PKL"), nullptr, L};
      a.eps_base = p.eps_base();
      a.stepn = x.stepn();
      SND_TRY(launch_reparam_fwd(a, x.s));
    }
    if (p.sg) SND_TRY(launch_sg_mean(x.f("ZL"), x.f("ZBAR"), p.B, p.S, L, x.s));
    {
      TrefProjFwdArgs a{x.f(p.sg ? "ZBAR" : "ZL"), p.B, L, x.w("dec.Wp"), x.w("dec.bp"), CP, x.f("Z")};
      SND_TRY(launch_tref_proj_fwd(a, x.s));
    }
    if (p.fast) {
      ReparamPrepArgs a{x.f("Z"), dj, N, zzt_npad(N), p.B, dj, nullptr, 0, nullptr, nullptr,
                        nullptr, (__bf16*)x.f("ZB"), (__bf16*)stg.jrow, (__bf16*)stg.jt, stg.colpart,
                        nullptr, 1};
      SND_TRY(launch_reparam_prep(a, zzt_dp(dj), x.s));
    }
  } else if (p.head_fused) {
    SND_TRY(head_fwd_fused(x, batch, eps, seed, step_counter, stg));
  } else if (p.fast) {
    ReparamPrepArgs a{x.f("MS"), 2 * L, N, zzt_npad(N), p.B, L, eps, seed, step_counter, x.f("Z"),
                      x.f("EPS"), (__bf16*)x.f("ZB"), (__bf16*)stg.jrow, (__bf16*)stg.jt, stg.colpart,
                      x.d("PKL")};
    a.eps_base = p.eps_base();
    a.stepn = x.stepn();
    SND_TRY(launch_reparam_prep(a, zzt_dp(L), x.s));
  } else {
    ReparamFwdArgs a{x.f("MS"), 2 * L, R, L, eps, seed, step_counter, x.f("EPS"), x.f("Z"),
                     x.d("PKL"), nullptr, L};
    a.eps_base = p.eps_base();
    a.stepn = x.stepn();
    SND_TRY(launch_reparam_fwd(a, x.s));
  }
  int edge_mark = -1;
  {
    SND_TRY(fork(x));
    if (p.head_bwd || p.edge_reparam) {
    } else if (p.fast) {
      EdgeBfArgs ea{rp, ci, R, (const __bf16*)x.f("ZB"), dj, c.pos_weight, x.f("EJ"), x.d("PEDGE"),
                    xcd_nbg(N, p.B)};
      ea.row_order = batch->row_order;
      SND_TRY(launch_edge_bf16(ea, side(x)));
    } else {
      EdgeArgs ea{rp, ci, R, x.f("Z"), dj, c.pos_weight, x.f("EJ"), x.d("PEDGE")};
// ... 99 lines not shown
      ReparamBwdArgs a{x.f("MS"), 2 * L, R, L, x.f("EPS"), x.f("DZDEC"), x.f("DJD"), x.f("EJ"),
                       adj_scale, kl_scale, x.f("DMS"), 2 * L};
      SND_TRY(launch_reparam_bwd(a, x.s));
    }
    if (!p.small_head) {
      SND_TRY(gemm_wgrad(x, x.f("Hh"), gh, gh, true, x.f("DMS"), 2 * L, 2 * L, x.f("SWMS"), p.sWms, RH));
      SND_TRY(gemm_fwd(x, RH, gh, 2 * L, x.f("DMS"), 2 * L, x.w("enc.Wms"), 2 * L, B_COL, x.f("DH"), gh,
                       nullptr));
    }
    if (p.sg) {
      SND_TRY(encoder_sg_bwd(x, batch));
    } else if (p.tref) {
      TrefHeadBwdArgs a{x.f("G"), KH, p.B, x.w("enc.Wh"), gh, x.f("DH"), x.g("enc.Wh"), x.f("DG")};
      if (p.fast_enc) {
        a.g = nullptr; a.dg = nullptr;
        a.gb = reinterpret_cast<const __bf16*>(x.f("FG")); a.ldg = p.ldg; a.W = W; a.npg = N;
        a.dgb = reinterpret_cast<__bf16*>(x.f("FDG"));
      }
      if (p.stream_fused("enc.Wh")) a.adam = fused_adam(x, "enc.Wh", step_counter);
      SND_TRY(launch_tref_head_bwd(a, x.s));
      if (p.ev_head && hipEventRecord(p.ev_head, x.s) != hipSuccess) {
        set_error("train step: grad event (enc.Wh) record failed");
        return SND_ERR_HIP;
      }
    } else {
      SND_TRY(gemm_wgrad(x, x.f("G"), W, W, true, x.f("DH"), gh, gh, x.f("SWH"), p.sWh));
      SND_TRY(gemm_fwd(x, R, W, gh, x.f("DH"), gh, x.w("enc.Wh"), gh, B_COL, x.f("DG"), W, nullptr));
    }
  }
  if (p.fast_enc && p.tref) {
    SND_TRY(encoder_fast_bwd_tail(x, batch));
  } else if (!p.fast_enc && !p.sg) {
    {
      EncBwdArgs a{x.f("DG"), W, x.f("H2"), W, x.w("enc.bne.gamma"), W, x.f("P1"), h1,
                   x.w("enc.bn1.gamma"), h1, x.f("DP1"), h1, x.f("PENC1"), 1};
      SND_TRY(launch_enc_bwd(a, R, x.s));
    }
    {
      SpmmArgs a{rp, ci, R, x.f("DP1"), h1, h1, x.f("DXW1"), h1, SND_SPMM_PLAIN};
      SND_TRY(launch_spmm(a, x.s));
    }
    SND_TRY(gemm_wgrad(x, x.f("H1"), h0 + f, h0 + f, false, x.f("DXW1"), h1, h1, x.f("SW1"), p.sW1));
    SND_TRY(gemm_fwd(x, R, h0, h1, x.f("DXW1"), h1, x.w("enc.W1"), h1, B_COL, x.f("DH1"), h0,
                     nullptr));
    {
      EncBwdArgs a{x.f("DH1"), h0, nullptr, 0, nullptr, 0, x.f("P0"), h0, x.w("enc.bn0.gamma"), h0,
                   x.f("DP0"), h0, x.f("PENC0"), 0};
      SND_TRY(launch_enc_bwd(a, R, x.s));
    }
    {
      SpmmArgs a{rp, ci, R, x.f("DP0"), h0, h0, x.f("DXW0"), h0, SND_SPMM_PLAIN};
      SND_TRY(launch_spmm(a, x.s));
    }
    SND_TRY(gemm_wgrad(x, X, f, f, false, x.f("DXW0"), h0, h0, x.f("SW0"), p.sW0));
  }

  SND_TRY(join(x));
  if (x.wq && !x.wq->empty()) {
    const bool k5n = !(debug_flags() & (1 << 25));
    auto key = [k5n](const WgArgs& u) {
      const long long c = (long long)u.T * u.K * u.N;
      return k5n && u.T == 5 && u.N <= 32 && u.K >= 32 ? 8 * c : c;
    };
    std::stable_sort(x.wq->begin(), x.wq->end(), [&](const WgArgs& u, const WgArgs& v) { return key(u) > key(v); });
    SND_TRY(launch_wgrad_multi(x.wq->data(), (int)x.wq->size(), x.s));
    p.last_wq = *x.wq;
  }

  std::vector<ReduceDesc> rd;
  final_reduce_descs(x, rd);
  const int nh = head_blocks(R);
  const int n_kl = (p.fast && !p.tref) ? reparam_prep_blocks(p.B, zzt_npad(N))
                   : (p.small_head ? small_head_fwd_blocks(L) : reparam_blocks(RH, L));
  FinalizeArgs fa{x.d("PZZT"), p.B * (zzt_npad(N) / 128) * (c.dtype == SND_BF16 ? x.zts : 1) * zzt_wpb(dj, c.dtype), x.d("PEDGE"),
                  p.head_bwd ? head_tiles(R) : (p.fast ? edge_bf16_blocks(R) : edge_blocks(R, dj)),
                  x.d("PKL"), n_kl, x.d(p.dec_fused ? "PDSSES" : "PSSES"),
                  x.d(p.dec_fused ? "PDSSEN" : "PSSEN"), p.dec_fused ? p.dtiles : nh,
                  rp, p.B, N, L, sd, nf, c.beta, c.norm, losses, grads + p.pcount, step_counter,
                  (double)RH * L};
  const unsigned long long amask = p.fuse_m ? reduce_adam_mask(p, rd, grads) : 0ull;
  if (amask) {
    SND_CHECK_ARG(step_counter && rd.size() <= 64, "train step: fused Adam needs the step counter");
    const ReduceAdam ra{grads, const_cast<float*>(params), p.fuse_m, p.fuse_v, p.fuse_lr, p.fuse_b1,
                        p.fuse_b2, p.fuse_eps, reinterpret_cast<const int*>(x.f("STEPN")), amask};
    return launch_reduce(rd.data(), (int)rd.size(), x.s, &fa, &ra);
  }
  return launch_reduce(rd.data(), (int)rd.size(), x.s, &fa);
}
```

snd_vae_amd/csrc/snd_tref.hip:

```cpp
#include "snd_tref.hpp"

#include <algorithm>

namespace snd {
namespace {

constexpr int B8 = kTrefMaxB;

__device__ __forceinline__ float4 f4(float a) { return make_float4(a, a, a, a); }
__device__ __forceinline__ void fma4(float4& acc, float s, const float4& w) {
  acc.x = fmaf(s, w.x, acc.x);
  acc.y = fmaf(s, w.y, acc.y);
  acc.z = fmaf(s, w.z, acc.z);
  acc.w = fmaf(s, w.w, acc.w);
}
__device__ __forceinline__ float dot4(const float4& a, const float4& b) {
  return fmaf(a.x, b.x, fmaf(a.y, b.y, fmaf(a.z, b.z, a.w * b.w)));
}

template <typename A>
__device__ __forceinline__ float g_at(const A& a, int b, long long k) {
  if (a.gb) {
    const long long n = k / a.W;
    return (float)a.gb[((long long)b * a.npg + n) * a.ldg + (k - n * a.W)];
  }
  return a.g[(long long)b * a.K + k];
}

__device__ __forceinline__ float4 ld_nt(const float* p) {
  const f32x4 v = __builtin_nontemporal_load(reinterpret_cast<const f32x4*>(p));
  return make_float4(v[0], v[1], v[2], v[3]);
}
__device__ __forceinline__ void st_nt(float* p, const float4& x) {
  const f32x4 v = {x.x, x.y, x.z, x.w};
  __builtin_nontemporal_store(v, reinterpret_cast<f32x4*>(p));
}

__device__ __forceinline__ float adam_lrt(const AdamFuse& f) {
  const int t = *f.step + 1;
  return (float)((double)f.lr * sqrt(1.0 - pow((double)f.b2, t)) / (1.0 - pow((double)f.b1, t)));
}
__device__ __forceinline__ void adam4(const AdamFuse& f, float lrt, long long i, const float4& g,
                                      float4 p, float4 m, float4 v) {
  adam_elem(p.x, m.x, v.x, g.x, f.b1, f.b2, f.eps, lrt);
  adam_elem(p.y, m.y, v.y, g.y, f.b1, f.b2, f.eps, lrt);
  adam_elem(p.z, m.z, v.z, g.z, f.b1, f.b2, f.eps, lrt);
  adam_elem(p.w, m.w, v.w, g.w, f.b1, f.b2, f.eps, lrt);
  st_nt(f.m + i, m);
  st_nt(f.v + i, v);
  st_nt(f.p + i, p);
}

constexpr int HF_T = 256;

__global__ void __launch_bounds__(HF_T) tref_head_fwd_kernel(TrefHeadFwdArgs a, int rpb) {
  extern __shared__ float sm[];
  const int TPR = a.gh >> 2, RPI = HF_T / TPR;
  const int t = threadIdx.x, q = t % TPR, r = t / TPR;
  const long long k0 = (long long)blockIdx.x * rpb;
  const int nk = (int)std::min<long long>(rpb, a.K - k0);
  for (int b = 0; b < B8; ++b)
    for (int kk = t; kk < nk; kk += HF_T)
      sm[kk * B8 + b] = b < a.B ? g_at(a, b, k0 + kk) : 0.f;
  __syncthreads();
  float4 acc[B8];
#pragma unroll
  for (int b = 0; b < B8; ++b) acc[b] = f4(0.f);
  if (r < RPI) {
    const float* wrow = a.wh + (k0 + r) * a.gh + 4 * q;
    const long long wstep = (long long)RPI * a.gh;
    int kk = r;
    for (; kk + 7 * RPI < nk; kk += 8 * RPI) {
      float4 w[8];
#pragma unroll
      for (int u = 0; u < 8; ++u) w[u] = *reinterpret_cast<const float4*>(wrow + u * wstep);
      wrow += 8 * wstep;
#pragma unroll
      for (int u = 0; u < 8; ++u) {
        const float4 g0 = *reinterpret_cast<const float4*>(sm + (kk + u * RPI) * B8);
        const float4 g1 = *reinterpret_cast<const float4*>(sm + (kk + u * RPI) * B8 + 4);
        fma4(acc[0], g0.x, w[u]); fma4(acc[1], g0.y, w[u]);
        fma4(acc[2], g0.z, w[u]); fma4(acc[3], g0.w, w[u]);
        fma4(acc[4], g1.x, w[u]); fma4(acc[5], g1.y, w[u]);
        fma4(acc[6], g1.z, w[u]); fma4(acc[7], g1.w, w[u]);
      }
    }
    float4 w[7];
#pragma unroll
    for (int u = 0; u < 7; ++u)
      w[u] = kk + u * RPI < nk ? *reinterpret_cast<const float4*>(wrow + u * wstep) : f4(0.f);
#pragma unroll
    for (int u = 0; u < 7; ++u) {
      if (kk + u * RPI >= nk) break;
      const float4 g0 = *reinterpret_cast<const float4*>(sm + (kk + u * RPI) * B8);
      const float4 g1 = *reinterpret_cast<const float4*>(sm + (kk + u * RPI) * B8 + 4);
      fma4(acc[0], g0.x, w[u]); fma4(acc[1], g0.y, w[u]); fma4(acc[2], g0.z, w[u]); fma4(acc[3], g0.w, w[u]);
      fma4(acc[4], g1.x, w[u]); fma4(acc[5], g1.y, w[u]); fma4(acc[6], g1.z, w[u]); fma4(acc[7], g1.w, w[u]);
    }
  }
  __syncthreads();
  if (r < RPI)
#pragma unroll
    for (int b = 0; b < B8; ++b)
      *reinterpret_cast<float4*>(sm + (r * B8 + b) * a.gh + 4 * q) = acc[b];
  __syncthreads();
  const int outs = a.B * a.gh;
  for (int o = t; o < outs; o += HF_T) {
    float s = 0.f;
    for (int rr = 0; rr < RPI; ++rr) s += sm[rr * B8 * a.gh + o];
    if (blockIdx.x == 0) s += a.bh[o % a.gh];
    a.slab[(long long)blockIdx.x * outs + o] = s;
  }
}

int head_fwd_rpb(long long K, int gh) {
  const int RPI = HF_T / (gh / 4);
  long long rpb = round_up(cdiv(K, 1024), RPI);
  rpb = std::max<long long>(rpb, 4LL * RPI);
  return (int)std::min<long long>(rpb, 1024);
}

constexpr int HB_T = 256, HB_RPB = 256;

// ... 143 lines not shown
  for (int i = t; i < a.L * B8; i += PB_T) {
    const int l = i >> 3, b = i & 7;
    zs[i] = b < a.B ? a.z[b * a.L + l] : 0.f;
  }
  const long long c4 = 4LL * ((long long)blockIdx.x * 64 + lane);
  const bool cv = c4 < a.Cp;
  float4 d[B8];
#pragma unroll
  for (int b = 0; b < B8; ++b) {
    d[b] = f4(0.f);
    if (cv && b < a.B) {
      const long long i = (long long)b * a.Cp + c4;
      const float4 x = *reinterpret_cast<const float4*>(a.dz_dec + i);
      const float4 y = *reinterpret_cast<const float4*>(a.dJd + i);
      const float4 z = *reinterpret_cast<const float4*>(a.ej + i);
      d[b] = make_float4(fmaf(a.adj_scale, y.x + z.x, x.x), fmaf(a.adj_scale, y.y + z.y, x.y),
                         fmaf(a.adj_scale, y.z + z.z, x.z), fmaf(a.adj_scale, y.w + z.w, x.w));
    }
  }
  if (wv == 0 && cv) {
    float4 s = d[0];
#pragma unroll
    for (int b = 1; b < B8; ++b) { s.x += d[b].x; s.y += d[b].y; s.z += d[b].z; s.w += d[b].w; }
    if (a.adam_b.p)
      adam4(a.adam_b, adam_lrt(a.adam_b), c4, s, ld_nt(a.adam_b.p + c4), ld_nt(a.adam_b.m + c4),
            ld_nt(a.adam_b.v + c4));
    else
      *reinterpret_cast<float4*>(a.dbp + c4) = s;
  }
  __syncthreads();
  const bool fused = a.adam.p != nullptr;
  const float lrt = fused ? adam_lrt(a.adam) : 0.f;
  constexpr int U = 5;
  for (int l0 = wv; l0 < a.L; l0 += PB_W * U) {
    float4 w[U], am[U], av[U];
#pragma unroll
    for (int u = 0; u < U; ++u) {
      const int l = l0 + PB_W * u;
      const bool ld = cv && l < a.L;
      const long long i = (long long)(ld ? l : 0) * a.Cp + (cv ? c4 : 0);
      w[u] = ld ? ld_nt(a.wp + i) : f4(0.f);
      am[u] = av[u] = f4(0.f);
      if (fused && ld) {
        am[u] = ld_nt(a.adam.m + i);
        av[u] = ld_nt(a.adam.v + i);
      }
    }
#pragma unroll
    for (int u = 0; u < U; ++u) {
      const int l = l0 + PB_W * u;
      if (l >= a.L) break;
      const float4 z0 = *reinterpret_cast<const float4*>(zs + l * B8);
      const float4 z1 = *reinterpret_cast<const float4*>(zs + l * B8 + 4);
      float4 dw = f4(0.f);
      fma4(dw, z0.x, d[0]); fma4(dw, z0.y, d[1]); fma4(dw, z0.z, d[2]); fma4(dw, z0.w, d[3]);
      fma4(dw, z1.x, d[4]); fma4(dw, z1.y, d[5]); fma4(dw, z1.z, d[6]); fma4(dw, z1.w, d[7]);
      if (cv) {
        if (fused) adam4(a.adam, lrt, (long long)l * a.Cp + c4, dw, w[u], am[u], av[u]);
        else *reinterpret_cast<float4*>(a.dwp + (long long)l * a.Cp + c4) = dw;
      }
#pragma unroll
      for (int b = 0; b < B8; ++b) {
        const float p = row16_sum(dot4(d[b], w[u]));
        if ((lane & 15) == 0) red[lane >> 4][l * B8 + b] = p;
      }
    }
  }
  __syncthreads();
  for (int i = t; i < a.L * a.B; i += PB_T) {
    const int b = i / a.L, l = i - b * a.L;
    const int j = l * B8 + b;
    a.slab[(long long)blockIdx.x * a.B * a.L + i] = (red[0][j] + red[1][j]) + (red[2][j] + red[3][j]);
  }
}

__global__ void __launch_bounds__(256) adam_vec_kernel(float4* p, const float4* g, float4* m,
                                                       float4* v, long long n4, float lr, float b1,
                                                       float b2, float eps, float gscale,
                                                       const int* step) {
  const long long i0 = (long long)blockIdx.x * 256 + threadIdx.x;
  const long long st = (long long)gridDim.x * 256;
  float4 gi, mi, vi, pi;
  if (i0 < n4) { gi = g[i0]; mi = m[i0]; vi = v[i0]; pi = p[i0]; }
  const int t = *step;
  const double lr_t = (double)lr * sqrt(1.0 - pow((double)b2, t)) / (1.0 - pow((double)b1, t));
  const float lrt = (float)lr_t;
  for (long long i = i0; i < n4; i += st) {
    if (i != i0) { gi = g[i]; mi = m[i]; vi = v[i]; pi = p[i]; }
    adam_elem(pi.x, mi.x, vi.x, __fmul_rn(gi.x, gscale), b1, b2, eps, lrt);
    adam_elem(pi.y, mi.y, vi.y, __fmul_rn(gi.y, gscale), b1, b2, eps, lrt);
    adam_elem(pi.z, mi.z, vi.z, __fmul_rn(gi.z, gscale), b1, b2, eps, lrt);
    adam_elem(pi.w, mi.w, vi.w, __fmul_rn(gi.w, gscale), b1, b2, eps, lrt);
    m[i] = mi;
    v[i] = vi;
    p[i] = pi;
  }
}

struct AdamRanges {
  long long off4[kAdamMaxRanges], start4[kAdamMaxRanges + 1];
  int n;
};
__global__ void __launch_bounds__(256) adam_ranges_kernel(float4* p, const float4* g, float4* m, float4* v,
                                                          AdamRanges rg, float lr, float b1, float b2,
                                                          float eps, float gscale, const int* step) {
  const long long tot = rg.start4[rg.n];
  const long long j = (long long)blockIdx.x * 256 + threadIdx.x;
  long long i = -1;
  if (j < tot) {
    int r = 0;
    while (r + 1 < rg.n && j >= rg.start4[r + 1]) ++r;
    i = rg.off4[r] + (j - rg.start4[r]);
  }
  float4 gi, mi, vi, pi;
  if (i >= 0) { gi = g[i]; mi = m[i]; vi = v[i]; pi = p[i]; }
  const int t = *step;
  const double lr_t = (double)lr * sqrt(1.0 - pow((double)b2, t)) / (1.0 - pow((double)b1, t));
  const float lrt = (float)lr_t;
  if (i < 0) return;
  adam_elem(pi.x, mi.x, vi.x, __fmul_rn(gi.x, gscale), b1, b2, eps, lrt);
  adam_elem(pi.y, mi.y, vi.y, __fmul_rn(gi.y, gscale), b1, b2, eps, lrt);
  adam_elem(pi.z, mi.z, vi.z, __fmul_rn(gi.z, gscale), b1, b2, eps, lrt);
  adam_elem(pi.w, mi.w, vi.w, __fmul_rn(gi.w, gscale), b1, b2, eps, lrt);
  m[i] = mi;
  v[i] = vi;
  p[i] = pi;
}

}

int launch_adam_ranges(float* p, const float* g, float* m, float* v, const long long* off,
                       const long long* cnt, int n, float lr, float b1, float b2, float eps, float gscale,
                       const int* step, hipStream_t s) {
  SND_CHECK_ARG(n >= 1 && n <= kAdamMaxRanges, "adam_ranges: 1..%d ranges", kAdamMaxRanges);
  SND_CHECK_ARG(((uintptr_t)p | (uintptr_t)g | (uintptr_t)m | (uintptr_t)v) % 16 == 0,
                "adam_ranges: 16-byte aligned buffers");
  AdamRanges rg{};
  rg.n = n;
  long long acc = 0;
  for (int k = 0; k < n; ++k) {
    SND_CHECK_ARG(off[k] >= 0 && cnt[k] >= 0 && off[k] % 4 == 0 && cnt[k] % 4 == 0,
                  "adam_ranges: offsets and counts must be multiples of 4");
    rg.off4[k] = off[k] / 4;
    rg.start4[k] = acc;
    acc += cnt[k] / 4;
  }
  rg.start4[n] = acc;
  if (acc == 0) return 0;
  hipLaunchKernelGGL(adam_ranges_kernel, dim3((unsigned)cdiv(acc, 256)), dim3(256), 0, s,
                     reinterpret_cast<float4*>(p), reinterpret_cast<const float4*>(g),
                     reinterpret_cast<float4*>(m), reinterpret_cast<float4*>(v), rg, lr, b1, b2, eps, gscale,
                     step);
  SND_LAUNCH_CHECK("adam_ranges_kernel");
  return 0;
}

int tref_head_fwd_blocks(long long K, int gh) { return cdiv(K, head_fwd_rpb(K, gh)); }

int launch_tref_head_fwd(const TrefHeadFwdArgs& a, hipStream_t s) {
  SND_CHECK_ARG(a.B >= 1 && a.B <= B8 && a.gh % 4 == 0 && a.gh >= 4 && a.gh <= 128 && a.K > 0,
                "tref_head_fwd: B in 1..8, g_hidden %% 4 in 4..128");
  SND_CHECK_ARG((a.g || (a.gb && a.W > 0 && a.npg > 0 && a.ldg >= a.W && (long long)a.W * a.npg == a.K)) &&
                    a.wh && a.bh && a.slab, "tref_head_fwd: null operand / bf16 G geometry");
  const int rpb = head_fwd_rpb(a.K, a.gh);
  const int RPI = HF_T / (a.gh / 4);
  const size_t lds = sizeof(float) * std::max<size_t>((size_t)rpb * B8, (size_t)RPI * B8 * a.gh);
  hipLaunchKernelGGL(tref_head_fwd_kernel, dim3(tref_head_fwd_blocks(a.K, a.gh)), dim3(HF_T), lds, s, a,
                     rpb);
  SND_LAUNCH_CHECK("tref_head_fwd_kernel");
  return 0;
}

int launch_tref_head_bwd(const TrefHeadBwdArgs& a, hipStream_t s) {
  SND_CHECK_ARG(a.B >= 1 && a.B <= B8 && a.gh % 4 == 0 && a.gh >= 4 && a.gh <= 128 && a.K > 0,
                "tref_head_bwd: B in 1..8, g_hidden %% 4 in 4..128");
  SND_CHECK_ARG((a.g || (a.gb && a.W > 0 && a.npg > 0 && a.ldg >= a.W && (long long)a.W * a.npg == a.K)) &&
                    a.wh && a.dh && (a.dwh || a.adam.p) && (a.dg || (a.dgb && a.gb)),
                "tref_head_bwd: null operand / bf16 G geometry");
  SND_CHECK_ARG(!a.adam.p || (a.adam.m && a.adam.v && a.adam.step && a.adam.p == a.wh),
                "tref_head_bwd: fused Adam needs m, v, step and p == wh");
  hipLaunchKernelGGL(tref_head_bwd_kernel, dim3(cdiv(a.K, HB_RPB)), dim3(HB_T), 0, s, a);
  SND_LAUNCH_CHECK("tref_head_bwd_kernel");
  return 0;
}

int launch_tref_proj_fwd(const TrefProjFwdArgs& a, hipStream_t s) {
  SND_CHECK_ARG(a.B >= 1 && a.B <= B8 && a.L >= 1 && a.L <= 128 && a.Cp % 4 == 0 && a.Cp > 0,
                "tref_proj_fwd: B in 1..8, L <= 128, Cp %% 4");
  SND_CHECK_ARG(a.z && a.wp && a.bp && a.j, "tref_proj_fwd: null operand");
  hipLaunchKernelGGL(tref_proj_fwd_kernel, dim3(cdiv(a.Cp / 4, 64)), dim3(64 * PF_W), 0, s, a);
  SND_LAUNCH_CHECK("tref_proj_fwd_kernel");
  return 0;
}

int tref_proj_bwd_blocks(long long Cp) { return cdiv(Cp, 256); }

int launch_tref_proj_bwd(const TrefProjBwdArgs& a, hipStream_t s) {
  SND_CHECK_ARG(a.B >= 1 && a.B <= B8 && a.L >= 1 && a.L <= 128 && a.Cp % 4 == 0 && a.Cp > 0,
                "tref_proj_bwd: B in 1..8, L <= 128, Cp %% 4");
  SND_CHECK_ARG(a.z && a.wp && a.dz_dec && a.dJd && a.ej && (a.dwp || a.adam.p) && (a.dbp || a.adam_b.p) &&
                    a.slab, "tref_proj_bwd: null operand");
// ... 25 lines not shown
```

Baseline: 39440 graphs/s.

## Precompute Adam step size in encoder blocks and hoist philox noise before head GEMMs

Adds an extra block to the gcn0/front encoder kernels that computes the Adam bias-corrected learning rate once into a workspace buffer. The fused reduce+Adam kernel then reads it instead of each block evaluating double-precision pow/sqrt. The head kernel now generates the philox reparameterisation noise before the GEMM stages, giving the RNG latency a chance to overlap with weight staging. Index math is also switched to shifts, which assumes L is a power of two. An optional 64-bit multiply philox variant is added but is off by default. The trade-offs are higher register pressure from holding the noise values and the extra launched block.

New measurement: 39690 graphs/s (median of 6 runs). Within noise of the previous version (+0.6%).

```diff
diff --git a/snd_vae_amd/csrc/snd_common.hpp b/snd_vae_amd/csrc/snd_common.hpp
--- a/snd_vae_amd/csrc/snd_common.hpp
+++ b/snd_vae_amd/csrc/snd_common.hpp
@@ -131,12 +131,22 @@
   return v;
 }
 
+#ifndef SND_PHILOX_MAD64
+#define SND_PHILOX_MAD64 0
+#endif
 __device__ __forceinline__ uint4 philox4x32_10(uint4 c, uint2 k) {
   const unsigned M0 = 0xD2511F53u, M1 = 0xCD9E8D57u, W0 = 0x9E3779B9u, W1 = 0xBB67AE85u;
 #pragma unroll
   for (int i = 0; i < 10; ++i) {
+#if SND_PHILOX_MAD64
+    unsigned long long p0 = (unsigned long long)M0 * c.x, p1 = (unsigned long long)M1 * c.z;
+    asm volatile("" : "+v"(p0), "+v"(p1));
+    const unsigned hi0 = (unsigned)(p0 >> 32), lo0 = (unsigned)p0;
+    const unsigned hi1 = (unsigned)(p1 >> 32), lo1 = (unsigned)p1;
+#else
     const unsigned hi0 = __umulhi(M0, c.x), lo0 = M0 * c.x;
     const unsigned hi1 = __umulhi(M1, c.z), lo1 = M1 * c.z;
+#endif
     c = make_uint4(hi1 ^ c.y ^ k.x, lo1, hi0 ^ c.w ^ k.y, lo0);
     k.x += W0;
     k.y += W1;
@@ -176,6 +186,13 @@
   dl = __fmaf_rn(__fmul_rn(dz, eps), es, __fmul_rn(kl, __fmaf_rn(es, es, -1.f)));
 }
 
+__device__ __forceinline__ float adam_lr_t_pw(float lr, double pb1, double pb2) {
+  return (float)((double)lr * sqrt(1.0 - pb2) / (1.0 - pb1));
+}
+__device__ __forceinline__ float adam_lr_t(float lr, float b1, float b2, int t) {
+  return adam_lr_t_pw(lr, pow((double)b1, t), pow((double)b2, t));
+}
+
 inline int cdiv(long long a, long long b) { return (int)((a + b - 1) / b); }
 inline long long round_up(long long a, long long b) { return (a + b - 1) / b * b; }
 
diff --git a/snd_vae_amd/csrc/snd_elem.hip b/snd_vae_amd/csrc/snd_elem.hip
--- a/snd_vae_amd/csrc/snd_elem.hip
+++ b/snd_vae_amd/csrc/snd_elem.hip
@@ -367,10 +367,7 @@
   const int bx = bid - pk.bstart[di];
   const bool dad = ADAM && ((ra.mask >> di) & 1ull);
   float lrt = 0.f;
-  if (dad) {
-    const int st = *ra.stepn;
-    lrt = (float)((double)ra.lr * sqrt(1.0 - pow((double)ra.b2, st)) / (1.0 - pow((double)ra.b1, st)));
-  }
+  if (dad && ra.lrt) lrt = *ra.lrt;
   __shared__ double red[256];
   const int rows = d.rows > 0 ? d.rows : 1;
   const long long items = (long long)rows * d.len;
@@ -427,6 +424,7 @@
     if constexpr (ADAM) {
       if (dad) {
         const long long k = dst - ra.gbase;
+        if (!ra.lrt) lrt = adam_lr_t(ra.lr, ra.b1, ra.b2, *ra.stepn);
         adam_elem(pi, mi, vi, __fmul_rn(v, 1.f), ra.b1, ra.b2, ra.eps, lrt);
         ra.m[k] = mi;
         ra.v[k] = vi;
@@ -485,9 +483,7 @@
 __global__ void __launch_bounds__(256) adam_kernel(float* p, const float* g, float* m, float* v,
                                                    long long n, float lr, float b1, float b2,
                                                    float eps, float gscale, const int* step) {
-  const int t = *step;
-  const double lr_t = (double)lr * sqrt(1.0 - pow((double)b2, t)) / (1.0 - pow((double)b1, t));
-  const float lrt = (float)lr_t;
+  const float lrt = adam_lr_t(lr, b1, b2, *step);
   for (long long i = (long long)blockIdx.x * 256 + threadIdx.x; i < n;
        i += (long long)gridDim.x * 256) {
     float pi = p[i], mi = m[i], vi = v[i];
diff --git a/snd_vae_amd/csrc/snd_fast.hpp b/snd_vae_amd/csrc/snd_fast.hpp
--- a/snd_vae_amd/csrc/snd_fast.hpp
+++ b/snd_vae_amd/csrc/snd_fast.hpp
@@ -26,6 +26,17 @@
   PackSrc s[2];
 };
 constexpr int kMaxPack = 16;
+struct LrtArgs {
+  float* out = nullptr;
+  const int* step = nullptr;
+  float lr = 0.f, b1 = 0.f, b2 = 0.f;
+};
+__device__ __forceinline__ void lrt_produce(const LrtArgs& l, double* pw) {
+  const int w = threadIdx.x >> 6;
+  if (w < 2 && (threadIdx.x & 63) == 0) pw[w] = pow((double)(w ? l.b2 : l.b1), *l.step + 1);
+  __syncthreads();
+  if (threadIdx.x == 0) *l.out = adam_lr_t_pw(l.lr, pw[0], pw[1]);
+}
 int launch_pack(const PackDesc* d, int n, hipStream_t s);
 size_t pack_bytes(int T, int kp, int np);
 
@@ -113,6 +124,7 @@
   int xcd_nbg;
   const int* row_order;
   PackDesc pack[kMaxPack]; int pack_blk[kMaxPack + 1]; int npack;
+  LrtArgs lrt;
 };
 int xcd_nbg(int npg, int ngraphs);
 int gcn0_blocks(int R);
diff --git a/snd_vae_amd/csrc/snd_fast_enc.hip b/snd_vae_amd/csrc/snd_fast_enc.hip
--- a/snd_vae_amd/csrc/snd_fast_enc.hip
+++ b/snd_vae_amd/csrc/snd_fast_enc.hip
@@ -25,8 +25,13 @@
 
 __global__ void __launch_bounds__(NT) gcn0_kernel(Gcn0Args a) {
   const int nrb = (a.R + RPB - 1) / RPB;
+  __shared__ __attribute__((aligned(16))) float sp[6][128];
   if ((int)blockIdx.x >= nrb) {
     const int pb = blockIdx.x - nrb;
+    if (pb >= a.pack_blk[a.npack]) {
+      lrt_produce(a.lrt, reinterpret_cast<double*>(&sp[0][0]));
+      return;
+    }
     int s = 0;
     while (s + 1 < a.npack && pb >= a.pack_blk[s + 1]) ++s;
     s = __builtin_amdgcn_readfirstlane(s);
@@ -35,7 +40,6 @@
     if (i < pack_chunks(d)) pack_chunk(d, i);
     return;
   }
-  __shared__ float sp[6][128];
   for (int i = threadIdx.x; i < a.h0; i += NT) {
 #pragma unroll
     for (int q = 0; q < 4; ++q) sp[q][i] = q < a.f ? a.w0[q * a.h0 + i] : 0.f;
@@ -737,7 +741,8 @@
                     a.ldh1 >= a.h0 + 8,
                 "gcn0: f in 1..4, h0 %% 8 (<= 128), ldh1 >= h0 + 8");
   SND_CHECK_ARG(a.rowptr && a.x && a.w0 && a.g0 && a.b0 && a.h1 && a.ax && a.axb, "gcn0: null operand");
-  hipLaunchKernelGGL(gcn0_kernel, dim3(gcn0_blocks(a.R) + pb), dim3(NT), 0, s, a);
+  SND_CHECK_ARG(!a.lrt.out || a.lrt.step, "gcn0: the step size needs the step counter");
+  hipLaunchKernelGGL(gcn0_kernel, dim3(gcn0_blocks(a.R) + pb + (a.lrt.out ? 1 : 0)), dim3(NT), 0, s, a);
   SND_LAUNCH_CHECK("gcn0_kernel");
   return 0;
 }
diff --git a/snd_vae_amd/csrc/snd_gemm.hpp b/snd_vae_amd/csrc/snd_gemm.hpp
--- a/snd_vae_amd/csrc/snd_gemm.hpp
+++ b/snd_vae_amd/csrc/snd_gemm.hpp
@@ -44,6 +44,7 @@
   float lr, b1, b2, eps;
   const int* stepn;
   unsigned long long mask;
+  const float* lrt = nullptr;
 };
 int launch_reduce(const ReduceDesc* d, int n, hipStream_t s, const FinalizeArgs* fin = nullptr,
                   const ReduceAdam* adam = nullptr);
diff --git a/snd_vae_amd/csrc/snd_head.hip b/snd_vae_amd/csrc/snd_head.hip
--- a/snd_vae_amd/csrc/snd_head.hip
+++ b/snd_vae_amd/csrc/snd_head.hip
@@ -97,6 +97,7 @@
   const int L = a.L, sxs = L + 4, zts = L + 1;
   const int tid = threadIdx.x, lane = tid & 63, w = tid >> 6;
   const int tpg = a.npad / HR;
+  const unsigned off = a.step ? (unsigned)(*a.step) : 0u;
   int tb = blockIdx.x;
   if (a.ngraphs % 8 == 0 && a.ngraphs > 0) {
     const int x = tb & 7, sq = tb >> 3;
@@ -133,6 +134,31 @@
   }
   stage_img(a.wh_img, a.np1 * a.kp1 * 2, reinterpret_cast<char*>(w1s), HW);
   stage_img(a.wms_img, a.np2 * a.kp2 * 2, reinterpret_cast<char*>(w2s), HW);
+  constexpr int NE = NB2 / 2;
+  float4 epq[NE];
+#pragma unroll
+  for (int k = 0; k < NE; ++k) epq[k] = make_float4(0.f, 0.f, 0.f, 0.f);
+  if (!(kdbg(a.dbg) & 32)) {
+    long long ie[NE];
+#pragma unroll
+    for (int k = 0; k < NE; ++k) {
+      const int it = tid + k * HT;
+      const int zr = it / (L >> 2), c = 4 * (it - zr * (L >> 2));
+      ie[k] = (gr0 + min(lr0 + zr, a.npg - 1)) * L + c;
+    }
+    if (!a.eps_in) {
+#pragma unroll
+      for (int k = 0; k < NE; ++k) {
+        epq[k] = philox_normal4(a.seed, off, (a.eps_base + (unsigned long long)ie[k]) >> 2);
+        asm volatile("" : "+v"(epq[k].x), "+v"(epq[k].y), "+v"(epq[k].z), "+v"(epq[k].w));
+      }
+    }
+    asm volatile("" ::: "memory");
+    if (a.eps_in) {
+#pragma unroll
+      for (int k = 0; k < NE; ++k) epq[k] = *reinterpret_cast<const float4*>(a.eps_in + ie[k]);
+    }
+  }
   if (tid < 128) {
     cb1[tid] = tid < a.gh ? bhv : 0.f;
     cb2[tid] = tid < 2 * L ? bmsv : 0.f;
@@ -220,7 +246,7 @@
 #pragma unroll
       for (int e = 0; e < 4; ++e) o[i][e] = acc2[i][e] + cb2[n0 + e];
       if (vrow && !(kdbg(a.dbg) & 8))
-        *reinterpret_cast<float4*>(a.ms + rr * (2 * L) + n0) = make_float4(o[i][0], o[i][1], o[i][2], o[i][3]);
+        *reinterpret_cast<float4*>(a.ms + (rr << (32 - __clz(L))) + n0) = make_float4(o[i][0], o[i][1], o[i][2], o[i][3]);
     }
     __syncthreads();
 #pragma unroll
@@ -233,22 +259,23 @@
   __syncthreads();
 
   {
-    const unsigned off = a.step ? (unsigned)(*a.step) : 0u;
     if (a.stepn && blockIdx.x == 0 && tid == 0) *a.stepn = (int)off + 1;
-    const int nq = L >> 2;
+    const int nq = L >> 2, lgL = 31 - __clz(L);
     double kl[HR / 64];
 #pragma unroll
     for (int h = 0; h < HR / 64; ++h) kl[h] = 0.0;
-    for (int it = (kdbg(a.dbg) & 32) ? HR * nq : tid; it < HR * nq; it += HT) {
-      const int zr = it / nq, c = 4 * (it - zr * nq);
+#pragma unroll
+    for (int k = 0; k < NE; ++k) {
+      if (kdbg(a.dbg) & 32) break;
+      const int it = tid + k * HT;
+      const int zr = it >> (lgL - 2), c = 4 * (it & (nq - 1));
       const int zl = lr0 + zr;
       float z4[4] = {0.f, 0.f, 0.f, 0.f};
       if (zl < a.npg) {
-        const long long ie = (gr0 + zl) * L + c;
+        const long long ie = ((gr0 + zl) << lgL) + c;
         const float4 m4 = *reinterpret_cast<const float4*>(mx + zr * sxs + c);
         const float4 s4 = *reinterpret_cast<const float4*>(sx + zr * sxs + c);
-        const float4 ep = a.eps_in ? *reinterpret_cast<const float4*>(a.eps_in + ie)
-                                   : philox_normal4(a.seed, off, (a.eps_base + (unsigned long long)ie) >> 2);
+        const float4 ep = epq[k];
         const float mu[4] = {m4.x, m4.y, m4.z, m4.w}, s[4] = {s4.x, s4.y, s4.z, s4.w};
         const float e[4] = {ep.x, ep.y, ep.z, ep.w};
         double kq = 0.0;
@@ -275,7 +302,7 @@
         jb[t] = (__bf16)(z4[t] * kSqrtLog2e);
         zt[zr * zts + c + t] = z4[t];
       }
-      *reinterpret_cast<bf16x4*>(a.jrow + ((long long)gi * a.npad + zl) * L + c) = jb;
+      *reinterpret_cast<bf16x4*>(a.jrow + (((long long)gi * a.npad + zl) << lgL) + c) = jb;
     }
 #pragma unroll
     for (int h = 0; h < HR / 64; ++h) {
@@ -285,7 +312,7 @@
   }
   __syncthreads();
   for (int i = (kdbg(a.dbg) & 64) ? HT * HR : tid; i < (HR / 64) * L; i += HT) {
-    const int h = i / L, c = i - h * L;
+    const int h = i >> (31 - __clz(L)), c = i & (L - 1);
     float cs = 0.f;
     for (int q0 = 0; q0 < 64; q0 += 16) {
       float t[16];
@@ -294,14 +321,14 @@
 #pragma unroll
       for (int u = 0; u < 16; ++u) cs += (float)(__bf16)(t[u] * kSqrtLog2e);
     }
-    a.colpart[((long long)gi * (a.npad / 64) + (HR / 64) * lt + h) * L + c] = cs;
+    a.colpart[(((long long)gi * (a.npad / 64) + (HR / 64) * lt + h) << (31 - __clz(L))) + c] = cs;
   }
   for (int idx = (kdbg(a.dbg) & 64) ? HT * HR : tid; idx < (HR / 4) * L; idx += HT) {
     const int c = idx / (HR / 4), r4 = 4 * (idx % (HR / 4));
     bf16x4 t;
 #pragma unroll
-    for (int u = 0; u < 4; ++u) t[u] = (__bf16)zt[(r4 + u) * zts + c];
-    *reinterpret_cast<bf16x4*>(a.jt + ((long long)gi * L + c) * a.npad + lr0 + r4) = t;
+    for (int u = 0; u < 4; ++u) t[u] = (__bf16)zt[((r4 + u) << (31 - __clz(L))) + r4 + u + c];
+    *reinterpret_cast<bf16x4*>(a.jt + (long long)gi * L * a.npad + c * a.npad + lr0 + r4) = t;
   }
   if (tid < HR / 64) {
     double v = 0.0;
@@ -700,8 +727,13 @@
 __global__ void __launch_bounds__(1024) enc_front_kernel(FrontArgs a) {
   const int tid = threadIdx.x;
   const int ntiles = cdiv_dev(a.R, 128);
+  extern __shared__ __attribute__((aligned(16))) char smem[];
   if ((int)blockIdx.x >= ntiles) {
     const int pb = blockIdx.x - ntiles;
+    if (pb >= a.pack_wg[a.npack]) {
+      lrt_produce(a.lrt, reinterpret_cast<double*>(smem));
+      return;
+    }
     int s = 0;
     while (s + 1 < a.npack && pb >= a.pack_wg[s + 1]) ++s;
     s = __builtin_amdgcn_readfirstlane(s);
@@ -710,7 +742,6 @@
     if (i < pack_chunks(d)) pack_chunk(d, i);
     return;
   }
-  extern __shared__ __attribute__((aligned(16))) char smem[];
   __shared__ float sp[6][128];
   __bf16* wimg = reinterpret_cast<__bf16*>(smem);
   __bf16* himg = reinterpret_cast<__bf16*>(smem + a.np1 * a.kp1 * 2);
@@ -866,7 +897,8 @@
   a.pack_wg[npack] = wg;
   SND_TRY(head_init_attributes());
   const size_t lds = (size_t)(a.np1 + 128) * a.kp1 * 2;
-  const dim3 grid(cdiv(a.R, 128) + wg);
+  SND_CHECK_ARG(!a.lrt.out || a.lrt.step, "front: the step size needs the step counter");
+  const dim3 grid(cdiv(a.R, 128) + wg + (a.lrt.out ? 1 : 0));
   switch ((a.np1 / 16 + 1) / 2) {
     case 1: hipLaunchKernelGGL((enc_front_kernel<1>), grid, dim3(1024), lds, s, a); break;
     case 2: hipLaunchKernelGGL((enc_front_kernel<2>), grid, dim3(1024), lds, s, a); break;
diff --git a/snd_vae_amd/csrc/snd_head.hpp b/snd_vae_amd/csrc/snd_head.hpp
--- a/snd_vae_amd/csrc/snd_head.hpp
+++ b/snd_vae_amd/csrc/snd_head.hpp
@@ -74,6 +74,7 @@
   __bf16* xw1;
   PackDesc pack[kMaxPack]; int npack;
   int pack_wg[kMaxPack + 1];
+  LrtArgs lrt;
   int dbg;
 };
 bool front_supported(int f, int h0, int n1, int kp1, int np1);
diff --git a/snd_vae_amd/csrc/snd_step.hip b/snd_vae_amd/csrc/snd_step.hip
--- a/snd_vae_amd/csrc/snd_step.hip
+++ b/snd_vae_amd/csrc/snd_step.hip
@@ -280,6 +280,7 @@
   const int nk = reparam_blocks(p->RH, L), nh = head_blocks(p->R), nc = col_blocks(p->R);
   p->add_buf("PZZT", 2LL * nz, 8); p->add_buf("PEDGE", 2LL * std::max({ne, edge_bf16_blocks(p->R), head_tiles(p->R)}), 8); p->add_buf("PKL", std::max({nk, reparam_prep_blocks(p->B, zzt_npad(p->N)), small_head_fwd_blocks(c.latent)}), 8);
   p->add_buf("STEPN", 1);
+  p->add_buf("LRT", 1);
   p->add_buf("PSSES", nh, 8); p->add_buf("PSSEN", nh, 8);
   p->add_buf("PHS", (long long)nh * (c.s3 * c.spatial_dim + c.spatial_dim));
   p->add_buf("PHN", (long long)nh * (c.n2 * c.num_feature + c.num_feature));
@@ -580,6 +581,7 @@
   const float* w(const char* n) const { return P + p->blk(n); }
   float* g(const char* n) const { return Gr + p->blk(n); }
   int* stepn() const { return reinterpret_cast<int*>(ws + p->buf("STEPN")); }
+  LrtArgs lrt;
 };
 
 AdamFuse fused_adam(const Ctx& x, const char* blk, const int* step) {
@@ -898,6 +900,7 @@
     a.h1 = bf("FH1"); a.ldh1 = p.ldh1; a.ax = x.f("AX"); a.axb = bf("AXB");
     a.w1 = x.w("enc.W1"); a.n1 = h1; a.kp1 = p.pw1f.kp; a.np1 = p.pw1f.np;
     a.xw1 = bf("FXW1"); a.dbg = debug_flags();
+    a.lrt = x.lrt;
     PackDesc e[kMaxPack]{};
     const int ne = build_packs(x, e);
     SND_TRY(launch_front(a, e, ne, x.s));
@@ -907,7 +910,7 @@
                x.w("enc.bn0.gamma"), x.w("enc.bn0.beta"), h0, bf("FH1"), p.ldh1, x.f("AX"), bf("AXB"),
                xcd_nbg(p.N, p.B)};
     a.row_order = batch->row_order;
-    if (p.pack_in_gcn0) a.npack = build_packs(x, a.pack);
+    if (p.pack_in_gcn0) { a.npack = build_packs(x, a.pack); a.lrt = x.lrt; }
     SND_TRY(launch_gcn0(a, x.s));
   }
   if (!p.front_fused) {
@@ -1605,6 +1608,8 @@
     wq.reserve(kMaxWgMulti);
     x.wq = &wq;
   }
+  if (p.fuse_m && step_counter && p.fast_enc && !p.sg && (p.front_fused || p.pack_in_gcn0))
+    x.lrt = LrtArgs{x.f("LRT"), step_counter, p.fuse_lr, p.fuse_b1, p.fuse_b2};
   const int R = p.R, N = p.N, f = c.f_in, h0 = c.h0, h1 = c.h1, gh = c.g_hidden, L = c.latent;
   const int W = p.W, C1 = p.C1, s1 = c.s1, s2 = c.s2, s3 = c.s3, n1 = c.n1, n2 = c.n2;
   const int sd = c.spatial_dim, nf = c.num_feature;
@@ -1870,7 +1875,7 @@
   if (amask) {
     SND_CHECK_ARG(step_counter && rd.size() <= 64, "train step: fused Adam needs the step counter");
     const ReduceAdam ra{grads, const_cast<float*>(params), p.fuse_m, p.fuse_v, p.fuse_lr, p.fuse_b1,
-                        p.fuse_b2, p.fuse_eps, reinterpret_cast<const int*>(x.f("STEPN")), amask};
+                        p.fuse_b2, p.fuse_eps, reinterpret_cast<const int*>(x.f("STEPN")), amask, x.lrt.out};
     return launch_reduce(rd.data(), (int)rd.size(), x.s, &fa, &ra);
   }
   return launch_reduce(rd.data(), (int)rd.size(), x.s, &fa);
diff --git a/snd_vae_amd/csrc/snd_tref.hip b/snd_vae_amd/csrc/snd_tref.hip
--- a/snd_vae_amd/csrc/snd_tref.hip
+++ b/snd_vae_amd/csrc/snd_tref.hip
@@ -37,8 +37,7 @@
 }
 
 __device__ __forceinline__ float adam_lrt(const AdamFuse& f) {
-  const int t = *f.step + 1;
-  return (float)((double)f.lr * sqrt(1.0 - pow((double)f.b2, t)) / (1.0 - pow((double)f.b1, t)));
+  return adam_lr_t(f.lr, f.b1, f.b2, *f.step + 1);
 }
 __device__ __forceinline__ void adam4(const AdamFuse& f, float lrt, long long i, const float4& g,
                                       float4 p, float4 m, float4 v) {
@@ -348,9 +347,7 @@
   const long long st = (long long)gridDim.x * 256;
   float4 gi, mi, vi, pi;
   if (i0 < n4) { gi = g[i0]; mi = m[i0]; vi = v[i0]; pi = p[i0]; }
-  const int t = *step;
-  const double lr_t = (double)lr * sqrt(1.0 - pow((double)b2, t)) / (1.0 - pow((double)b1, t));
-  const float lrt = (float)lr_t;
+  const float lrt = adam_lr_t(lr, b1, b2, *step);
   for (long long i = i0; i < n4; i += st) {
     if (i != i0) { gi = g[i]; mi = m[i]; vi = v[i]; pi = p[i]; }
     adam_elem(pi.x, mi.x, vi.x, __fmul_rn(gi.x, gscale), b1, b2, eps, lrt);
@@ -380,9 +377,7 @@
   }
   float4 gi, mi, vi, pi;
   if (i >= 0) { gi = g[i]; mi = m[i]; vi = v[i]; pi = p[i]; }
-  const int t = *step;
-  const double lr_t = (double)lr * sqrt(1.0 - pow((double)b2, t)) / (1.0 - pow((double)b1, t));
-  const float lrt = (float)lr_t;
+  const float lrt = adam_lr_t(lr, b1, b2, *step);
   if (i < 0) return;
   adam_elem(pi.x, mi.x, vi.x, __fmul_rn(gi.x, gscale), b1, b2, eps, lrt);
   adam_elem(pi.y, mi.y, vi.y, __fmul_rn(gi.y, gscale), b1, b2, eps, lrt);
```
